# LorenzoFramba/Continual-Learning

Measured on AMD Instinct MI355X. Metric: images/sec UNET 256x256 bs16 train step, higher is better.
Workload: dtype f32; 1 GPU; UNet(21,3,64) 256x256 bs16/GPU fp32 train step (fwd + CE + bwd + Adam), BASELINE.json configs[1]; global_batch=16, parallelism=dp1

## Files before the change

### continual-learning_amd/_lib.py

```python
import ctypes
import os
from ctypes import c_char_p, c_double, c_int, c_longlong, c_size_t, c_void_p

_HERE = os.path.dirname(os.path.abspath(__file__))
LIB_PATH = os.environ.get('CLAMD_LIB') or os.path.join(_HERE, 'libclamd.so')

F32, BF16, SPLIT = 0, 1, 2
WGRAD_CONV3, WGRAD_PW, WGRAD_UP2 = 0, 1, 2

_P, _I, _D, _LL, _SZ = c_void_p, c_int, c_double, c_longlong, c_size_t
OP_CONV3X3, OP_CONV3X3_WINOGRAD, OP_CONV1X1, OP_CONVT2X2_DGRAD, OP_BN_BWD_REDUCE, OP_CONV3X3_WINOGRAD24, OP_CONV3X3_WINOGRAD44 = range(7)


class Tuning(ctypes.Structure):
    _fields_ = [(n, c_int) for n in ('igemm_pws', 'igemm_ws', 'igemm_variant', 'pws_wres', 'wgrad_ws', 'wgrad_dma',
                                     'wgrad_xcd', 'wgrad_blocks', 'wgrad_tw16', 'wino_band', 'wino_persist', 'wino_mt',
                                     'bn_reduce_blocks', 'chsum_blocks', 'cu_reserve', 'wino_half', 'wgrad_streamk')] + [('reserved', c_int * 7)]

    def __init__(self, **kw):
        super().__init__()
        load().clamd_tuning_init(ctypes.byref(self))
        for k, v in kw.items():
            if k not in dict(self._fields_):
                raise KeyError(f'unknown tuning field {k!r}')
            setattr(self, k, int(v))

    def ref(self):
        return ctypes.addressof(self)

    def as_dict(self):
        return {n: getattr(self, n) for n, _ in self._fields_ if n != 'reserved'}


def tune_ptr(t):
    return None if t is None else t.ref()


SIGNATURES = {
    'clamd_last_error': (c_char_p, []),
    'clamd_version': (_I, []),
    'clamd_sizeof_pack_job': (_I, []),
    'clamd_sizeof_adam_tensor': (_I, []),
    'clamd_adam_chunk_elems': (_I, []),
    'clamd_sizeof_importance_tensor': (_I, []),
    'clamd_pack_tile': (_I, []),
    'clamd_bn_bwd_nsums': (_I, []),
    'clamd_sizeof_tuning': (_I, []),
    'clamd_tuning_init': (None, [_P]),
    'clamd_stat_rows': (_I, [_I, _I, _I, _I, _I, _I, _I, _I, _P]),
    'clamd_conv3x3': (_I, [_P, _I, _P, _P, _P, _I, _P, _P, _P, _I, _I, _I, _I, _I, _I, _I, _I, _I, _P, _P]),
    'clamd_conv3x3_border_bias_ok': (_I, [_I, _I, _I, _I, _I, _I, _P]),
    'clamd_conv3x3_bn_sums': (_I, [_I, _I, _I, _I, _I, _I, _P]),
    'clamd_bn_fold_bias': (_I, [_P, _P, _P, _P, _I, _I, _I, _P]),
    'clamd_maxpool2x2': (_I, [_P, _I, _P, _P, _I, _I, _I, _I, _I, _I, _P]),
    'clamd_maxpool2x2_bwd': (_I, [_P, _I, _P, _P, _I, _P, _I, _I, _I, _I, _I, _I, _P]),
    'clamd_bn_fold_pack': (_I, [_I, _P, _I, _I, _I, _P, _I, _P, _P, _P, _I, _I, _I, _P]),
    'clamd_bn_fold_wgrad_pointwise': (_I, [_P, _P, _P, _P, _I, _I, _P]),
    'clamd_bn_fold_wgrad_workspace_bytes': (_SZ, [_I, _I]),
    'clamd_bn_fold_wgrad': (_I, [_P, _I, _P, _P, _P, _P, _P, _SZ, _I, _I, _I, _I, _I, _I, _I, _P]),
    'clamd_conv1x1': (_I, [_P, _I, _P, _P, _P, _I, _P, _P, _P, _I, _I, _I, _I, _I, _I, _I, _I, _P]),
    'clamd_conv1x1_logits': (_I, [_P, _I, _P, _P, _P, _I, _I, _I, _I, _I, _I, _I, _P]),
    'clamd_conv1x1_argmax': (_I, [_P, _I, _P, _P, _P, _P, _I, _I, _I, _I, _I, _I, _I, _P]),
    'clamd_convT2x2_fwd': (_I, [_P, _I, _P, _P, _P, _I, _I, _I, _I, _I, _I, _I, _P]),
    'clamd_convT2x2_dgrad': (_I, [_P, _I, _P, _P, _I, _P, _P, _I, _I, _I, _I, _I, _I, _I, _P]),
    'clamd_wgrad_workspace_bytes': (_SZ, [_I, _I, _I, _I, _I, _I, _I]),
    'clamd_wgrad': (_I, [_I, _P, _I, _P, _I, _P, _SZ, _P, _I, _I, _I, _I, _I, _I, _I, _I, _I, _I, _I, _I, _P, _P]),
    'clamd_bn_finalize': (_I, [_P, _I, _P, _P, _P, _P, _P, _P, _P, _P, _I, _I, _D, _D, _D, _P, _P]),
    'clamd_bn_apply': (_I, [_P, _I, _P, _P, _P, _I, _P, _I, _I, _I, _I, _I, _I, _P]),
    'clamd_bn_bwd_reduce': (_I, [_P, _I, _P, _I, _P, _I, _P, _P, _P, _I, _I, _I, _I, _I, _I, _P, _P]),
    'clamd_bn_bwd_finalize': (_I, [_P, _I, _P, _P, _P, _P, _P, _P, _P, _I, _I, _D, _P]),
    'clamd_bn_bwd_apply': (_I, [_P, _I, _P, _I, _P, _I, _P, _P, _P, _P, _I, _I, _I, _I, _I, _I, _P]),
    'clamd_bn_bwd_apply_sums_rows': (_I, [_I, _I, _I, _I]),
    'clamd_bn_bwd_apply_sums': (_I, [_P, _I, _P, _I, _P, _P, _I, _P, _I, _I, _I, _I, _I, _I, _P]),
    'clamd_rows_sum': (_I, [_P, _I, _P, _I, _I, _P]),
    'clamd_bn_bwd_eval_rows': (_I, [_I, _I, _I, _I, _I]),
    'clamd_bn_bwd_eval': (_I, [_P, _I, _P, _I, _P, _I, _P, _P, _P, _I, _P, _I, _I, _I, _I, _I, _I, _I, _P]),
    'clamd_bn_bwd_eval_finalize': (_I, [_P, _I, _I, _P, _P, _P, _P, _P, _P, _P, _I, _I, _P]),
    'clamd_bn_rows_total': (_I, [_P, _I, _I, _I, _D, _P, _P, _P]),
    'clamd_bn_finalize_total': (_I, [_P, _P, _P, _P, _P, _P, _P, _P, _P, _I, _I, _D, _D, _P, _P]),
    'clamd_bn_bwd_finalize_total': (_I, [_P, _P, _P, _P, _P, _P, _P, _P, _P, _I, _I, _P]),
    'clamd_channel_sum_workspace_bytes': (_SZ, [_I]),
    'clamd_channel_sum': (_I, [_P, _I, _P, _LL, _I, _I, _I, _P, _SZ, _P, _P]),
    'clamd_nchw_to_nhwc': (_I, [_P, _P, _I, _I, _I, _I, _I, _I, _D, _I, _P]),
    'clamd_nhwc_to_nchw': (_I, [_P, _I, _P, _I, _I, _I, _I, _I, _P]),
    'clamd_nchw_im2col3': (_I, [_P, _P, _I, _I, _I, _I, _I, _I, _I, _P]),
    'clamd_pack': (_I, [_P, _I, _I, _I, _P]),
    'clamd_sizeof_wino_pack_job': (_I, []),
    'clamd_wino_pack': (_I, [_P, _I, _I, _P]),
    'clamd_wgrad_winograd_workspace_bytes': (_SZ, [_I, _I]),
    'clamd_wgrad_winograd24_workspace_bytes': (_SZ, [_I, _I]),
    'clamd_wgrad_winograd24': (_I, [_P, _I, _P, _I, _P, _SZ, _P, _I, _I, _I, _I, _I, _I, _I, _I, _I, _I, _I, _P, _P]),
    'clamd_wgrad_winograd': (_I, [_P, _I, _P, _I, _P, _SZ, _P, _I, _I, _I, _I, _I, _I, _I, _I, _I, _I, _I, _P, _P]),
    'clamd_conv3x3_winograd': (_I, [_P, _I, _P, _P, _P, _I, _P, _I, _I, _I, _I, _I, _I, _I, _P, _P]),
    'clamd_wino24_pack': (_I, [_P, _I, _I, _P]),
    'clamd_conv3x3_winograd24': (_I, [_P, _I, _P, _P, _P, _I, _P, _I, _I, _I, _I, _I, _I, _I, _P, _P]),
    'clamd_winograd24_input_elems': (_SZ, [_I, _I, _I, _I]),
    'clamd_winograd24_transform_input': (_I, [_P, _I, _P, _P, _P, _I, _I, _I, _I, _P]),
    'clamd_conv3x3_winograd24_pre': (_I, [_P, _P, _P, _P, _I, _P, _I, _I, _I, _I, _I, _I, _I, _P, _P]),
    'clamd_conv3x3_winograd24_direct_filters': (_I, [_P, _I, _P, _P, _P, _I, _P, _I, _I, _I, _I, _I, _I, _I, _P, _P]),
    'clamd_wgrad_winograd24_pre_operand_elems': (_SZ, [_I, _I, _I, _I]),
    'clamd_wgrad_winograd24_pre_transform': (_I, [_P, _I, _P, _I, _I, _I, _I, _P]),
    'clamd_wgrad_winograd24_pre_workspace_bytes': (_SZ, [_I, _I, _I, _I, _I]),
    'clamd_wgrad_winograd24_pre': (_I, [_P, _I, _P, _P, _P, _SZ, _P, _I, _I, _I, _I, _I, _I, _I, _I, _I, _I, _I, _P, _P]),
    'clamd_wino44_pack': (_I, [_P, _I, _I, _P]),
    'clamd_winograd44_input_elems': (_SZ, [_I, _I, _I, _I]),
    'clamd_winograd44_transform_input': (_I, [_P, _I, _P, _P, _P, _I, _I, _I, _I, _P]),
    'clamd_conv3x3_winograd44_pre': (_I, [_P, _P, _P, _P, _I, _P, _I, _I, _I, _I, _I, _I, _I, _P, _P]),
    'clamd_wgrad_winograd44_pre_operand_elems': (_SZ, [_I, _I, _I, _I]),
    'clamd_wgrad_winograd44_pre_transform': (_I, [_P, _I, _P, _I, _I, _I, _I, _P]),
    'clamd_wgrad_winograd44_pre_workspace_bytes': (_SZ, [_I, _I, _I, _I, _I]),
    'clamd_wgrad_winograd44_pre': (_I, [_P, _I, _P, _P, _P, _SZ, _P, _I, _I, _I, _I, _I, _I, _I, _I, _I, _I, _I, _P, _P]),
    'clamd_ce_workspace_bytes': (_SZ, []),
    'clamd_ce_bad_label_count_offset': (_SZ, []),
    'clamd_ce_fwd_bwd': (_I, [_P, _P, _P, _I, _I, _D, _D, _P, _P, _P, _SZ, _I, _I, _I, _I, _LL, _D, _P]),
    'clamd_ce_count': (_I, [_P, _I, _I, _I, _I, _LL, _P, _SZ, _P]),
    'clamd_ce_fwd_bwd_counted': (_I, [_P, _P, _P, _P, _I, _I, _P, _P, _SZ, _I, _I, _I, _I, _LL, _D, _P]),
    'clamd_ce_unbiased_fwd_bwd': (_I, [_P, _P, _P, _I, _I, _D, _P, _P, _I, _I, _P, _P, _SZ, _I, _I, _I, _I, _LL, _D, _P]),
    'clamd_ce_dice_workspace_bytes': (_SZ, [_I, _I, _I, _I, _I]),
    'clamd_ce_dice_fwd_bwd': (_I, [_P, _P, _P, _P, _I, _I, _P, _P, _SZ, _I, _I, _I, _I, _LL, _D, _D, _D, _I, _I, _I, _D, _P]),
    'clamd_pseudo_entropy_hist': (_I, [_P, _I, _I, _P, _P, _I, _I, _I, _I, _P]),
    'clamd_pseudo_label': (_I, [_P, _I, _I, _P, _P, _P, _P, _P, _D, _I, _I, _I, _LL, _P]),
    'clamd_ce_fwd_bwd_weighted': (_I, [_P, _P, _P, _P, _P, _I, _I, _P, _P, _SZ, _I, _I, _I, _I, _LL, _D, _P]),
    'clamd_pod_workspace_bytes': (_SZ, [_I, _I, _I, _I, _I]),
    'clamd_local_pod_fwd_bwd': (_I, [_P, _I, _P, _I, _I, _I, _I, _I, _I, _D, _P, _P, _P, _SZ, _I, _I, _I, _D, _P]),
    'clamd_class_pixel_counts': (_I, [_P, _P, _P, _I, _I, _I, _I, _LL, _P]),
    'clamd_replay_store': (_I, [_P, _P, _P, _P, _I, _P, _P, _I, _I, _P, _I, _I, _I, _I, _I, _LL, _P]),
    'clamd_replay_mix': (_I, [_P, _P, _I, _P, _P, _I, _I, _P, _P, _I, _P, _P, _P, _I, _I, _I, _LL, _P]),
    'clamd_augment_batch': (_I, [_P, _P, _P, _I, _I, _I, _I, _P, _P, _D, _LL, _P, _P]),
    'clamd_adam_step': (_I, [_P, _P, _I, _P, _P, _P, _P, _P]),
    'clamd_adam_step_consolidated': (_I, [_P, _P, _P, _I, _P, _P, _P, _P, _P, _P]),
    'clamd_importance_accum': (_I, [_P, _P, _I, _D, _D, _I, _P]),
    'clamd_sizeof_sgd_tensor': (_I, []),
    'clamd_sgd_step': (_I, [_P, _P, _P, _I, _P, _P, _P, _P]),
    'clamd_adam_step_tracked': (_I, [_P, _P, _P, _P, _I, _P, _P, _P, _P, _P, _P]),
    'clamd_sgd_step_tracked': (_I, [_P, _P, _P, _P, _I, _P, _P, _P, _P]),
    'clamd_sizeof_path_tensor': (_I, []),
    'clamd_path_importance': (_I, [_P, _P, _I, _D, _D, _P]),
    'clamd_argmax_confusion': (_I, [_P, _P, _P, _P, _I, _I, _I, _I, _I, _P]),
    'clamd_voc_prepare': (_I, [_P, _P, _P, _P, _I, _I, _I, _I, _I, _I, _P, _P]),
    'clamd_label_to_rgb': (_I, [_P, _P, _LL, _LL, _P]),
    'clamd_fill_f32': (_I, [_P, _LL, _D, _P]),
    'clamd_hold_cus': (_I, [_I, _I, _P]),
    'clamd_f32_to_bf16': (_I, [_P, _P, _LL, _P]),
    'clamd_bf16_to_f32': (_I, [_P, _P, _LL, _P]),
    'clamd_scale_by_device_scalar': (_I, [_P, _LL, _P, _P]),
    'clamd_scale_by_device_scalar_nhwc': (_I, [_P, _LL, _I, _P, _P, _LL, _P]),
}

DEBUG_SIGNATURES = {'clamd_debug_hold_cus': (_I, [_I, _I, _P]), 'clamd_debug_mfma_rate': (_LL, [_I, _I, _P, _P])}

_lib = None


def load():
# ... 61 lines not shown
```

### continual-learning_amd/csrc/elementwise.hip

```cpp
#include <initializer_list>
#include <type_traits>
#include "common.hip.h"
#include "clamd_internal.h"

namespace clamd {


constexpr int FIN_THREADS = 256, FIN_CH = 2;
template <int NK>
__device__ inline void sum_partial_rows(const float* __restrict__ rows, int nrows, int Cp, int c0, double* red, double* out) {
    constexpr int COLS = NK * FIN_CH, RL = FIN_THREADS / COLS;
    const int t = threadIdx.x, col = t % COLS, rl = t / COLS;
    if (rl < RL) {
        const float* p = rows + (size_t)(col / FIN_CH) * Cp + c0 + (col % FIN_CH);
        const size_t rs = (size_t)NK * Cp;
        double a0 = 0., a1 = 0., a2 = 0., a3 = 0.;
        int r = rl;
        for (; r + 3 * RL < nrows; r += 4 * RL) {
            a0 += (double)p[(size_t)r * rs]; a1 += (double)p[(size_t)(r + RL) * rs];
            a2 += (double)p[(size_t)(r + 2 * RL) * rs]; a3 += (double)p[(size_t)(r + 3 * RL) * rs];
        }
        for (; r < nrows; r += RL) a0 += (double)p[(size_t)r * rs];
        red[rl * COLS + col] = (a0 + a1) + (a2 + a3);
    }
    __syncthreads();
    if (t < COLS) {
        double v = 0.;
        for (int q = 0; q < RL; ++q) v += red[q * COLS + t];
        out[t] = v;
    }
    __syncthreads();
}

__device__ inline void bn_finalize_channel(bool stats, double s0, double s1, double count, int c, int C, const float* __restrict__ gamma,
                                           const float* __restrict__ beta, float* running_mean, float* running_var, float* scale,
                                           float* shift, float* save_mean, float* save_istd, double momentum, double eps) {
    double mean, var;
    if (stats) {
        mean = s0 / count;
        var = s1 / count - mean * mean;
        var = var > 0. ? var : 0.;
    } else {
        mean = c < C ? (double)running_mean[c] : 0.;
        var = c < C ? (double)running_var[c] : 1.;
    }
    const double istd = 1.0 / sqrt(var + eps);
    const double g = c < C ? (double)gamma[c] : 0., b = c < C ? (double)beta[c] : 0.;
    const float sc = (float)(g * istd);
    scale[c] = sc;
    shift[c] = (float)(b - mean * (g * istd));
    save_mean[c] = (float)mean;
    save_istd[c] = (float)istd;
    if (c < C && running_mean && stats) {
        const double unb = count > 1. ? var * (count / (count - 1.)) : var;
        running_mean[c] = (float)((1. - momentum) * (double)running_mean[c] + momentum * mean);
        running_var[c] = (float)((1. - momentum) * (double)running_var[c] + momentum * unb);
    }
}

__global__ void __launch_bounds__(FIN_THREADS) bn_finalize_kernel(const float* __restrict__ stats, int nrows, const float* __restrict__ gamma,
                                   const float* __restrict__ beta, float* running_mean, float* running_var,
                                   float* scale, float* shift, float* save_mean, float* save_istd,
                                   int Cp, int C, double count, double momentum, double eps, long long* num_batches_tracked) {
    PASS_PRIO();
    __shared__ double red[FIN_THREADS], tot[2 * FIN_CH];
    const int c0 = blockIdx.x * FIN_CH;
    if (stats) sum_partial_rows<2>(stats, nrows, Cp, c0, red, tot);
    if (threadIdx.x >= FIN_CH) return;
    if (num_batches_tracked && stats && blockIdx.x == 0 && threadIdx.x == 0) *num_batches_tracked += 1;
    const int c = c0 + threadIdx.x;
    bn_finalize_channel(stats != nullptr, stats ? tot[threadIdx.x] : 0., stats ? tot[FIN_CH + threadIdx.x] : 0., count, c, C, gamma, beta,
                        running_mean, running_var, scale, shift, save_mean, save_istd, momentum, eps);
}

template <int NK>
__global__ void __launch_bounds__(FIN_THREADS) bn_rows_total_kernel(const float* __restrict__ rows, int nrows, int Cp, double count,
                                                                    double* totals, double* reduce) {
    PASS_PRIO();
    __shared__ double red[FIN_THREADS], tot[NK * FIN_CH];
    const int c0 = blockIdx.x * FIN_CH;
    sum_partial_rows<NK>(rows, nrows, Cp, c0, red, tot);
    if (threadIdx.x >= NK * FIN_CH) return;
    const int k = threadIdx.x / FIN_CH, c = c0 + threadIdx.x % FIN_CH;
    const double v = tot[threadIdx.x];
    if (totals) totals[(size_t)k * Cp + c] = v;
    if (reduce && k < 2) reduce[(size_t)k * Cp + c] = v;
// ... 50 lines not shown
    Vec8<T>::load(ga + pix1 * ga_ldc + cg * 8, g[1]);
    Vec8<T>::load(y + pix1 * y_ldc + cg * 8, v[1]);
    return two;
}

template <typename T, bool POOL>
__global__ void bn_apply_kernel(const T* __restrict__ y, int y_ldc, const float* __restrict__ scale,
                                const float* __restrict__ shift, T* out, int out_ldc, T* pooled, int p_ldc,
                                int B, int H, int W, int Cp) {
    PASS_PRIO();
    const int G = Cp >> 3;
    const long long nitem = POOL ? (long long)B * (H / 2) * (W / 2) * G : (long long)B * H * W * G;
    const long long it0 = (long long)blockIdx.x * blockDim.x + threadIdx.x;
    const int cg = (int)(it0 % G);
    float sc[8], sh[8];
#pragma unroll
    for (int j = 0; j < 8; ++j) { sc[j] = scale[cg * 8 + j]; sh[j] = shift[cg * 8 + j]; }
    for (long long it = it0; it < nitem; it += (long long)gridDim.x * blockDim.x) {
        const long long pix = it / G;
        if constexpr (!POOL) {
            float v[8];
            Vec8<T>::load(y + pix * y_ldc + cg * 8, v);
#pragma unroll
            for (int j = 0; j < 8; ++j) v[j] = __fmaf_rn(v[j], sc[j], sh[j]);
            Vec8<T>::store(out + pix * out_ldc + cg * 8, v);
        } else {
            const PoolWindow win(pix, H, W);
            float m[8];
#pragma unroll
            for (int q = 0; q < 4; ++q) {
                const long long p = win.at(q);
                float v[8];
                Vec8<T>::load(y + p * y_ldc + cg * 8, v);
#pragma unroll
                for (int j = 0; j < 8; ++j) {
                    v[j] = __fmaf_rn(v[j], sc[j], sh[j]);
                    m[j] = (q == 0 || v[j] > m[j]) ? v[j] : m[j];
                }
                Vec8<T>::store(out + p * out_ldc + cg * 8, v);
            }
            Vec8<T>::store(pooled + pix * p_ldc + cg * 8, m);
        }
    }
}

template <typename T, bool BWD>
__global__ void __launch_bounds__(256) maxpool2x2_kernel(const T* __restrict__ x, int x_ldc, T* __restrict__ out, int o_ldc,
                                                        const T* __restrict__ gp, int gp_ldc, const float* __restrict__ sign,
                                                        int B, int H, int W, int Cp) {
    PASS_PRIO();
    const int G = Cp >> 3;
    const long long nitem = (long long)B * (H / 2) * (W / 2) * G;
    for (long long it = (long long)blockIdx.x * blockDim.x + threadIdx.x; it < nitem; it += (long long)gridDim.x * blockDim.x) {
        const int cg = (int)(it % G);
        const long long pix = it / G;
        const PoolWindow win(pix, H, W);
        float m[8], v[4][8];
        int arg[8];
        bool neg[8];
#pragma unroll
        for (int j = 0; j < 8; ++j) neg[j] = sign != nullptr && sign[cg * 8 + j] < 0.f;
#pragma unroll
        for (int q = 0; q < 4; ++q) {
            Vec8<T>::load(x + win.at(q) * x_ldc + cg * 8, v[q]);
#pragma unroll
            for (int j = 0; j < 8; ++j)
                if (q == 0 || (neg[j] ? v[q][j] < m[j] : v[q][j] > m[j])) { m[j] = v[q][j]; arg[j] = q; }
        }
        if constexpr (!BWD) Vec8<T>::store(out + pix * o_ldc + cg * 8, m);
        else {
            float g[8];
            Vec8<T>::load(gp + pix * gp_ldc + cg * 8, g);
#pragma unroll
            for (int q = 0; q < 4; ++q) {
                float o[8];
#pragma unroll
                for (int j = 0; j < 8; ++j) o[j] = arg[j] == q ? g[j] : 0.f;
                Vec8<T>::store(out + win.at(q) * o_ldc + cg * 8, o);
            }
        }
    }
}

template <typename T>
__device__ inline void load_gu(const T* ga, int ga_ldc, const T* gp, int gp_ldc, const T* y, int y_ldc,
                               const float (&sc)[8], const float (&sh)[8], const PoolWindow& win,
                               int cg, float (&g)[4][8], float (&yy)[4][8]) {
    float best[8];
    int arg[8];
#pragma unroll
    for (int q = 0; q < 4; ++q) {
        const long long p = win.at(q);
        Vec8<T>::load(y + p * y_ldc + cg * 8, yy[q]);
        if (ga) Vec8<T>::load(ga + p * ga_ldc + cg * 8, g[q]);
        else {
#pragma unroll
            for (int j = 0; j < 8; ++j) g[q][j] = 0.f;
        }
#pragma unroll
        for (int j = 0; j < 8; ++j) {
            float u = __fmaf_rn(yy[q][j], sc[j], sh[j]);
            if (q == 0 || u > best[j]) { best[j] = u; arg[j] = q; }
        }
    }
    float gpv[8];
    Vec8<T>::load(gp + win.cell() * gp_ldc + cg * 8, gpv);
#pragma unroll
    for (int q = 0; q < 4; ++q)
#pragma unroll
        for (int j = 0; j < 8; ++j) g[q][j] += (arg[j] == q) ? gpv[j] : 0.f;
}

constexpr int NSUM = 5;

__device__ inline void add_five_sums(float (&acc)[NSUM][8], const float (&g)[8], const float (&v)[8]) {
#pragma unroll
    for (int j = 0; j < 8; ++j) {
        const float pos = v[j] > 0.f ? 1.f : 0.f;
        acc[0][j] += g[j]; acc[1][j] += g[j] * v[j]; acc[2][j] += g[j] * pos;
        acc[3][j] += pos; acc[4][j] += v[j];
    }
}

template <typename T, bool POOL>
__global__ void __launch_bounds__(256) bn_bwd_reduce_kernel(const T* __restrict__ ga, int ga_ldc,
                                                            const T* __restrict__ gp, int gp_ldc,
                                                            const T* __restrict__ y, int y_ldc,
                                                            const float* __restrict__ scale,
                                                            const float* __restrict__ shift, float* sums,
                                                            int B, int H, int W, int Cp) {
    PASS_PRIO();
    __shared__ float red[256 * 8];
    const int G = Cp >> 3;
    const int tid = threadIdx.x;
    float acc[NSUM][8];
#pragma unroll
    for (int s = 0; s < NSUM; ++s)
#pragma unroll
        for (int j = 0; j < 8; ++j) acc[s][j] = 0.f;
    const int cg = tid % G;
    const int rows = 256 / G, prow = tid / G;
    {
        float sc[8], sh[8];
        if constexpr (POOL) {
#pragma unroll
            for (int j = 0; j < 8; ++j) { sc[j] = scale[cg * 8 + j]; sh[j] = shift[cg * 8 + j]; }
        }
        const long long npix = POOL ? (long long)B * (H / 2) * (W / 2) : (long long)B * H * W;
        const long long stride = (long long)gridDim.x * rows;
        for (long long pix = (long long)blockIdx.x * rows + prow; pix < npix; pix += POOL ? stride : 2 * stride) {
            if constexpr (!POOL) {
                float g[2][8], v[2][8];
                const bool two = pix + stride < npix;
                const long long pix1 = two ? pix + stride : pix;
                Vec8<T>::load(ga + pix * ga_ldc + cg * 8, g[0]);
                Vec8<T>::load(y + pix * y_ldc + cg * 8, v[0]);
                Vec8<T>::load(ga + pix1 * ga_ldc + cg * 8, g[1]);
                Vec8<T>::load(y + pix1 * y_ldc + cg * 8, v[1]);
#pragma unroll
                for (int u = 0; u < 2; ++u) {
                    if (u == 1 && !two) break;
#pragma unroll
                    for (int j = 0; j < 8; ++j) {
                        const float pos = v[u][j] > 0.f ? 1.f : 0.f;
                        acc[0][j] += g[u][j]; acc[1][j] += g[u][j] * v[u][j]; acc[2][j] += g[u][j] * pos;
                        acc[3][j] += pos; acc[4][j] += v[u][j];
                    }
                }
            } else {
                float g[4][8], v[4][8];
                load_gu<T>(ga, ga_ldc, gp, gp_ldc, y, y_ldc, sc, sh, PoolWindow(pix, H, W), cg, g, v);
#pragma unroll
                for (int q = 0; q < 4; ++q) add_five_sums(acc, g[q], v[q]);
            }
        }
    }
    float* dst = sums + (size_t)blockIdx.x * NSUM * Cp;
    if constexpr (POOL) reduce_block_rows<NSUM>(acc, red, dst, G, Cp, rows);
    else {
#pragma unroll
        for (int s = 0; s < NSUM; ++s) {
            __syncthreads();
#pragma unroll
            for (int j = 0; j < 8; ++j) red[tid * 8 + j] = acc[s][j];
            __syncthreads();
            for (int c = tid; c < Cp; c += 256) {
                const int g8 = c >> 3, j = c & 7;
                float t = 0.f;
                for (int r = 0; r < rows; ++r) t += red[(r * G + g8) * 8 + j];
                dst[s * Cp + c] = t;
            }
        }
    }
// ... 19 lines not shown

__global__ void __launch_bounds__(FIN_THREADS) bn_bwd_finalize_kernel(const float* __restrict__ sums, int nrows, const float* __restrict__ gamma,
                                       const float* __restrict__ save_mean, const float* __restrict__ save_istd,
                                       float* k012, float* dgamma, float* dbeta, float* dbias, int Cp, int C,
                                       double count) {
    PASS_PRIO();
    __shared__ double red[FIN_THREADS], tot[NSUM * FIN_CH];
    const int c0 = blockIdx.x * FIN_CH;
    sum_partial_rows<NSUM>(sums, nrows, Cp, c0, red, tot);
    if (threadIdx.x >= FIN_CH) return;
    const int c = c0 + threadIdx.x;
    double s[NSUM];
#pragma unroll
    for (int k = 0; k < NSUM; ++k) s[k] = tot[k * FIN_CH + threadIdx.x];
    bn_bwd_finalize_channel(s[0], s[1], count, s[0], s[1], s[2], s[3], s[4], c, C, Cp, gamma, save_mean, save_istd, k012, dgamma, dbeta, dbias);
}

__global__ void __launch_bounds__(256) bn_bwd_finalize_total_kernel(const double* __restrict__ totals, const double* __restrict__ reduce,
                                                                    const float* __restrict__ gamma, const float* __restrict__ save_mean,
                                                                    const float* __restrict__ save_istd, float* k012, float* dgamma,
                                                                    float* dbeta, float* dbias, int Cp, int C) {
    PASS_PRIO();
    const int c = blockIdx.x * blockDim.x + threadIdx.x;
    if (c >= Cp) return;
    const double* t = totals + c;
    const double s2 = dbias ? t[2 * (size_t)Cp] : 0., s3 = dbias ? t[3 * (size_t)Cp] : 0., s4 = dbias ? t[4 * (size_t)Cp] : 0.;
    bn_bwd_finalize_channel(reduce[c], reduce[Cp + c], reduce[2 * Cp], t[0], t[Cp], s2, s3, s4, c, C, Cp, gamma, save_mean, save_istd,
                            k012, dgamma, dbeta, dbias);
}

__device__ inline float bn_bwd_gz(float k0, float k1, float k2, float g, float y) { return fmaf(k0, g, fmaf(k1, y, k2)); }


__device__ inline void load_k012(const float* k012, int Cp, int cg, float (&k0)[8], float (&k1)[8], float (&k2)[8]) {
#pragma unroll
    for (int j = 0; j < 8; ++j) {
        k0[j] = k012[cg * 8 + j]; k1[j] = k012[Cp + cg * 8 + j]; k2[j] = k012[2 * Cp + cg * 8 + j];
    }
}

template <typename T, bool POOL>
__global__ void bn_bwd_apply_kernel(const T* __restrict__ ga, int ga_ldc, const T* __restrict__ gp, int gp_ldc,
                                    const T* __restrict__ y, int y_ldc, const float* __restrict__ scale,
                                    const float* __restrict__ shift, const float* __restrict__ k012, T* gz,
                                    int gz_ldc, int B, int H, int W, int Cp) {
    PASS_PRIO();
    const int G = Cp >> 3;
    const long long nitem = POOL ? (long long)B * (H / 2) * (W / 2) * G : (long long)B * H * W * G;
    const long long it0 = (long long)blockIdx.x * blockDim.x + threadIdx.x;
    float k0[8], k1[8], k2[8];
    if constexpr (!POOL) {
        const int cg = (int)(it0 % G);
        load_k012(k012, Cp, cg, k0, k1, k2);
        for (long long it = it0; it < nitem; it += (long long)gridDim.x * blockDim.x) {
            const long long pix = it / G;
            float g[8], v[8];
            Vec8<T>::load(ga + pix * ga_ldc + cg * 8, g);
            Vec8<T>::load(y + pix * y_ldc + cg * 8, v);
#pragma unroll
            for (int j = 0; j < 8; ++j) g[j] = v[j] > 0.f ? bn_bwd_gz(k0[j], k1[j], k2[j], g[j], v[j]) : 0.f;
            Vec8<T>::store(gz + pix * gz_ldc + cg * 8, g);
        }
    } else {
        for (long long it = it0; it < nitem; it += (long long)gridDim.x * blockDim.x) {
            const int cg = (int)(it % G);
            const long long pix = it / G;
            load_k012(k012, Cp, cg, k0, k1, k2);
            float sc[8], sh[8];
#pragma unroll
            for (int j = 0; j < 8; ++j) { sc[j] = scale[cg * 8 + j]; sh[j] = shift[cg * 8 + j]; }
            const PoolWindow win(pix, H, W);
            float g[4][8], v[4][8];
            load_gu<T>(ga, ga_ldc, gp, gp_ldc, y, y_ldc, sc, sh, win, cg, g, v);
#pragma unroll
            for (int q = 0; q < 4; ++q) {
#pragma unroll
                for (int j = 0; j < 8; ++j) g[q][j] = v[q][j] > 0.f ? bn_bwd_gz(k0[j], k1[j], k2[j], g[q][j], v[q][j]) : 0.f;
                Vec8<T>::store(gz + win.at(q) * gz_ldc + cg * 8, g[q]);
            }
        }
    }
}

template <typename T>
__global__ void __launch_bounds__(256) bn_bwd_apply_sums_kernel(const T* __restrict__ ga, int ga_ldc, const T* __restrict__ y, int y_ldc,
                                                                const float* __restrict__ k012, T* gz, int gz_ldc, float* rows,
                                                                long long npix, int Cp) {
    PASS_PRIO();
    __shared__ float red[256 * 8];
    const int G = Cp >> 3;
    const long long nitem = npix * G;
    const long long it0 = (long long)blockIdx.x * 256 + threadIdx.x;
    const int cg = (int)(it0 % G);
    float k0[8], k1[8], k2[8], acc[1][8] = {};
    load_k012(k012, Cp, cg, k0, k1, k2);
    for (long long it = it0; it < nitem; it += (long long)gridDim.x * 256) {
        const long long pix = it / G;
        float g[8], v[8];
        Vec8<T>::load(ga + pix * ga_ldc + cg * 8, g);
        Vec8<T>::load(y + pix * y_ldc + cg * 8, v);
#pragma unroll
        for (int j = 0; j < 8; ++j) {
            g[j] = v[j] > 0.f ? bn_bwd_gz(k0[j], k1[j], k2[j], g[j], v[j]) : 0.f;
            acc[0][j] += g[j];
        }
        Vec8<T>::store(gz + pix * gz_ldc + cg * 8, g);
    }
    reduce_block_rows<1>(acc, red, rows + (size_t)blockIdx.x * Cp, G, Cp, 256 / G);
}

constexpr int NSUM_EVAL = 3;

__device__ inline void add_eval_sums(float (&acc)[NSUM_EVAL][8], const float (&sc)[8], int nlive, float (&g)[8], const float (&v)[8]) {
#pragma unroll
    for (int j = 0; j < 8; ++j) {
        const float o = (v[j] > 0.f && j < nlive) ? sc[j] * g[j] : 0.f;
        acc[0][j] += g[j]; acc[1][j] += g[j] * v[j]; acc[2][j] += o;
        g[j] = o;
    }
}

template <typename T, bool POOL>
__global__ void __launch_bounds__(256) bn_bwd_eval_kernel(const T* __restrict__ ga, int ga_ldc, const T* __restrict__ gp, int gp_ldc,
                                                          const T* __restrict__ y, int y_ldc, const float* __restrict__ scale,
                                                          const float* __restrict__ shift, T* __restrict__ gz, int gz_ldc, float* rows,
                                                          int B, int H, int W, int Cp, int C) {
    PASS_PRIO();
    __shared__ float red[256 * 8];
    const int G = Cp >> 3, tid = threadIdx.x;
    const int cg = tid % G, prow = tid / G, per = 256 / G;
    const int nlive = C - cg * 8;
    float sc[8], acc[NSUM_EVAL][8];
#pragma unroll
    for (int j = 0; j < 8; ++j) {
        sc[j] = scale[cg * 8 + j];
#pragma unroll
        for (int s = 0; s < NSUM_EVAL; ++s) acc[s][j] = 0.f;
    }
    const long long npix = POOL ? (long long)B * (H / 2) * (W / 2) : (long long)B * H * W;
    const long long stride = (long long)gridDim.x * per;
    if constexpr (!POOL) {
        for (long long pix = (long long)blockIdx.x * per + prow; pix < npix; pix += 2 * stride) {
            float g[2][8], v[2][8];
            long long pix1;
            const bool two = load_pixel_pair<T>(ga, ga_ldc, y, y_ldc, pix, stride, npix, cg, pix1, g, v);
            add_eval_sums(acc, sc, nlive, g[0], v[0]);
            Vec8<T>::store(gz + pix * gz_ldc + cg * 8, g[0]);
            if (two) {
                add_eval_sums(acc, sc, nlive, g[1], v[1]);
                Vec8<T>::store(gz + pix1 * gz_ldc + cg * 8, g[1]);
            }
        }
    } else {
        float sh[8];
#pragma unroll
        for (int j = 0; j < 8; ++j) sh[j] = shift[cg * 8 + j];
        for (long long pix = (long long)blockIdx.x * per + prow; pix < npix; pix += stride) {
            const PoolWindow win(pix, H, W);
            float g[4][8], v[4][8];
            load_gu<T>(ga, ga_ldc, gp, gp_ldc, y, y_ldc, sc, sh, win, cg, g, v);
#pragma unroll
            for (int q = 0; q < 4; ++q) {
#pragma unroll
                for (int j = 0; j < 8; ++j) {
                    const float o = (v[q][j] > 0.f && j < nlive) ? sc[j] * g[q][j] : 0.f;
                    acc[0][j] += g[q][j]; acc[1][j] += g[q][j] * v[q][j]; acc[2][j] += o;
// ... 206 lines not shown
        }
        Vec8<T>::store(dst + pix * ldc + cg * 8, o);
    }
}

template <typename T>
__global__ void nhwc_to_nchw_kernel(const T* __restrict__ src, int ldc, float* dst, int B, int C, int H, int W) {
    const long long hw = (long long)H * W, n = (long long)B * C * hw;
    for (long long it = (long long)blockIdx.x * blockDim.x + threadIdx.x; it < n;
         it += (long long)gridDim.x * blockDim.x) {
        const long long p = it % hw;
        const int c = (int)((it / hw) % C);
        const long long b = it / (hw * C);
        dst[it] = ld1<T>(src + (b * hw + p) * ldc + c);
    }
}

static inline long long reduce_grid_cap(int forced, int Cp, int lo, int hi, int budget) {
    if (forced > 0) return forced;
    long long c = budget / Cp;
    return c < lo ? lo : (c > hi ? hi : c);
}

}

using namespace clamd;

static inline long long grid_rows(long long items, long long per, long long cap) {
    const long long g = (items + per - 1) / per;
    return g > cap ? cap : (g < 1 ? 1 : g);
}
static inline int ew_grid(long long nitem, int cap = 4096) { return (int)grid_rows(nitem, 256, cap); }
static bool pow2_channels(int Cp) { return Cp >= 32 && Cp <= 2048 && (Cp & (Cp - 1)) == 0; }
static const char POW2_RULE[] = "physical channels must be a power of two in [32,2048]";
static inline long long pass_pixels(int B, int H, int W, bool pooled) { return pooled ? (long long)B * (H / 2) * (W / 2) : (long long)B * H * W; }
static inline int pixel_rows(int Cp) { return 256 / (Cp / 8) > 0 ? 256 / (Cp / 8) : 1; }

long long clamd_bn_bwd_reduce_rows(int B, int H, int W, int Cp, bool pooled, const clamd_tuning& tn) {
    return grid_rows(pass_pixels(B, H, W, pooled), pixel_rows(Cp), reduce_grid_cap(tn.bn_reduce_blocks, Cp, 256, 1024, 131072));
}
constexpr int CHSUM_MAX_BLOCKS = 1024;

template <typename T> struct Tag { using type = T; };
template <typename F>
static bool dispatch(int dtype, bool flag, F&& f) {
    auto with_flag = [&](auto tag) { if (flag) f(tag, std::true_type{}); else f(tag, std::false_type{}); };
    if (dtype == CLAMD_BF16) with_flag(Tag<bf16_t>{});
    else if (dtype == CLAMD_F32) with_flag(Tag<float>{});
    else if (dtype == CLAMD_SPLIT) with_flag(Tag<split_t>{});
    else return false;
    return true;
}
template <typename F>
static bool dispatch(int dtype, F&& f) { return dispatch(dtype, false, [&](auto tag, auto) { f(tag); }); }

static int fail(const char* name, const char* text) {
    static thread_local char msg[256];
    snprintf(msg, sizeof(msg), "%s: %s", name, text);
    return clamd_fail(msg);
}

enum Need { OPTIONAL, REQUIRED, SOURCE };
constexpr int NO_PITCH = 0x7fffffff;
struct TensorArg { const void* p; int ldc; Need need; };
static int check_streaming(const char* name, bool channels_ok, const char* channel_rule, int Cp, long long B, long long H, long long W,
                           bool pooled, int dtype, std::initializer_list<TensorArg> tensors) {
    if (!channels_ok) return fail(name, channel_rule);
    if (B <= 0 || H <= 0 || W <= 0) return fail(name, "bad sizes");
    if (pooled && ((H | W) & 1)) return fail(name, "pooling needs even H, W");
    bool has_source = false, any_source = false;
    for (const TensorArg& t : tensors) {
        if (t.need == REQUIRED && !t.p) return fail(name, "null argument");
        if (t.need == SOURCE) { any_source = true; has_source |= t.p != nullptr; }
    }
    if (any_source && !has_source) return fail(name, "no gradient source (ga and gp are both a null argument)");
    for (const TensorArg& t : tensors)
        if (t.p && t.ldc < Cp) return fail(name, "pitches must be >= Cp");
    for (const TensorArg& t : tensors)
        if (t.ldc != NO_PITCH)
            if (int e = clamd_check_split(dtype, t.p, t.ldc)) return e;
    return 0;
}

extern "C" {

int clamd_bn_finalize(const float* stats, int stat_rows, const float* gamma, const float* beta, float* running_mean,
                      float* running_var, float* scale, float* shift, float* save_mean, float* save_istd,
                      int Cp, int C, double count, double momentum, double eps, long long* num_batches_tracked, void* stream) {
    if (Cp <= 0 || Cp % 8 || C > Cp) return clamd_fail("bn_finalize: bad channel counts");
    if (stats && stat_rows <= 0) return clamd_fail("bn_finalize: stat_rows must be the row count the producing launch wrote");
    if (!scale || !shift || !save_mean || !save_istd || (C > 0 && (!gamma || !beta))) return clamd_fail("bn_finalize: null argument");
    if (!stats && C > 0 && (!running_mean || !running_var)) return clamd_fail("bn_finalize: eval mode (stats == NULL) needs the running statistics");
    if (!running_mean != !running_var) return clamd_fail("bn_finalize: running_mean and running_var go together");
    hipLaunchKernelGGL(bn_finalize_kernel, dim3(Cp / FIN_CH), dim3(FIN_THREADS), 0, (hipStream_t)stream, stats, stat_rows, gamma,
                       beta, running_mean, running_var, scale, shift, save_mean, save_istd, Cp, C, count, momentum, eps, num_batches_tracked);
    return clamd_check_launch("bn_finalize");
}

int clamd_bn_rows_total(const float* rows, int nrows, int nk, int Cp, double count, double* totals, double* reduce, void* stream) {
    if (Cp <= 0 || Cp % 8) return clamd_fail("bn_rows_total: bad channel count");
    if (!rows || nrows <= 0) return clamd_fail("bn_rows_total: nrows must be the row count the producing launch wrote");
    if (!totals && !reduce) return clamd_fail("bn_rows_total: nothing to write");
    if (!(count > 0.)) return clamd_fail("bn_rows_total: count must be positive");
    hipStream_t s = (hipStream_t)stream;
    if (nk == 2)
        hipLaunchKernelGGL(bn_rows_total_kernel<2>, dim3(Cp / FIN_CH), dim3(FIN_THREADS), 0, s, rows, nrows, Cp, count, totals, reduce);
    else if (nk == NSUM)
        hipLaunchKernelGGL(bn_rows_total_kernel<NSUM>, dim3(Cp / FIN_CH), dim3(FIN_THREADS), 0, s, rows, nrows, Cp, count, totals, reduce);
    else return clamd_fail("bn_rows_total: nk must be 2 (statistics rows) or 5 (clamd_bn_bwd_nsums rows)");
    return clamd_check_launch("bn_rows_total");
}

int clamd_bn_finalize_total(const double* reduce, const float* gamma, const float* beta, float* running_mean, float* running_var,
                            float* scale, float* shift, float* save_mean, float* save_istd, int Cp, int C, double momentum, double eps,
                            long long* num_batches_tracked, void* stream) {
    if (Cp <= 0 || Cp % 8 || C <= 0 || C > Cp) return clamd_fail("bn_finalize_total: bad channel counts");
    if (!reduce || !gamma || !beta || !scale || !shift || !save_mean || !save_istd) return clamd_fail("bn_finalize_total: null argument");
    if (!running_mean != !running_var) return clamd_fail("bn_finalize_total: running_mean and running_var go together");
    hipLaunchKernelGGL(bn_finalize_total_kernel, dim3((Cp + 255) / 256), dim3(256), 0, (hipStream_t)stream, reduce, gamma, beta, running_mean,
                       running_var, scale, shift, save_mean, save_istd, Cp, C, momentum, eps, num_batches_tracked);
    return clamd_check_launch("bn_finalize_total");
}

int clamd_bn_apply(const void* y, int y_ldc, const float* scale, const float* shift, void* out, int out_ldc,
                   void* pooled, int p_ldc, int B, int H, int W, int Cp, int dtype, void* stream) {
    if (int e = check_streaming("bn_apply", pow2_channels(Cp), POW2_RULE, Cp, B, H, W, pooled != nullptr, dtype,
                                {{y, y_ldc, REQUIRED}, {scale, NO_PITCH, REQUIRED}, {shift, NO_PITCH, REQUIRED}, {out, out_ldc, REQUIRED},
                                 {pooled, p_ldc, OPTIONAL}}))
        return e;
    const dim3 g(ew_grid(pass_pixels(B, H, W, pooled != nullptr) * (Cp / 8), 8192)), b(256);
    const bool ok = dispatch(dtype, pooled != nullptr, [&](auto tag, auto pool) {
        using T = typename decltype(tag)::type;
        hipLaunchKernelGGL((bn_apply_kernel<T, decltype(pool)::value>), g, b, 0, (hipStream_t)stream, (const T*)y, y_ldc, scale, shift,
                           (T*)out, out_ldc, (T*)pooled, p_ldc, B, H, W, Cp);
    });
    return ok ? clamd_check_launch("bn_apply") : fail("bn_apply", "bad dtype");
}

static int launch_maxpool(const char* name, bool bwd, const void* x, int x_ldc, void* out, int o_ldc, const void* gp, int gp_ldc,
                          const float* sign, int B, int H, int W, int Cp, int dtype, void* stream) {
    if (int e = check_streaming(name, Cp > 0 && Cp % 8 == 0, "physical channels must be a positive multiple of 8", Cp, B, H, W, true, dtype,
                                {{x, x_ldc, REQUIRED}, {out, o_ldc, REQUIRED}, {gp, gp_ldc, bwd ? REQUIRED : OPTIONAL}}))
        return e;
    const dim3 g(ew_grid(pass_pixels(B, H, W, true) * (Cp / 8), 8192)), b(256);
    const bool ok = dispatch(dtype, bwd, [&](auto tag, auto back) {
        using T = typename decltype(tag)::type;
        hipLaunchKernelGGL((maxpool2x2_kernel<T, decltype(back)::value>), g, b, 0, (hipStream_t)stream, (const T*)x, x_ldc, (T*)out, o_ldc,
                           (const T*)gp, gp_ldc, sign, B, H, W, Cp);
    });
    return ok ? clamd_check_launch(name) : fail(name, "bad dtype");
}

int clamd_maxpool2x2(const void* x, int x_ldc, const float* sign, void* pooled, int p_ldc, int B, int H, int W, int Cp, int dtype, void* stream) {
    return launch_maxpool("maxpool2x2", false, x, x_ldc, pooled, p_ldc, nullptr, 0, sign, B, H, W, Cp, dtype, stream);
}

int clamd_maxpool2x2_bwd(const void* x, int x_ldc, const float* sign, const void* gp, int gp_ldc, void* gx, int gx_ldc, int B, int H, int W, int Cp,
                         int dtype, void* stream) {
    return launch_maxpool("maxpool2x2_bwd", true, x, x_ldc, gx, gx_ldc, gp, gp_ldc, sign, B, H, W, Cp, dtype, stream);
}

int clamd_bn_bwd_reduce(const void* ga, int ga_ldc, const void* gp, int gp_ldc, const void* y, int y_ldc,
                        const float* scale, const float* shift, float* sums, int sum_rows, int B, int H, int W, int Cp,
                        int dtype, const clamd_tuning* tune, void* stream) {
    const Need pool_only = gp ? REQUIRED : OPTIONAL;
    if (int e = check_streaming("bn_bwd_reduce", pow2_channels(Cp), POW2_RULE, Cp, B, H, W, gp != nullptr, dtype,
                                {{ga, ga_ldc, SOURCE}, {gp, gp_ldc, SOURCE}, {y, y_ldc, REQUIRED}, {sums, NO_PITCH, REQUIRED},
                                 {scale, NO_PITCH, pool_only}, {shift, NO_PITCH, pool_only}}))
        return e;
    if (int e = clamd_check_tuning(tune)) return e;
    const long long nrows = clamd_bn_bwd_reduce_rows(B, H, W, Cp, gp != nullptr, clamd_tune(tune));
    if (sum_rows != nrows) return fail("bn_bwd_reduce", "sum_rows does not match clamd_stat_rows(CLAMD_OP_BN_BWD_REDUCE, ...)");
    const bool ok = dispatch(dtype, gp != nullptr, [&](auto tag, auto pool) {
        using T = typename decltype(tag)::type;
        hipLaunchKernelGGL((bn_bwd_reduce_kernel<T, decltype(pool)::value>), dim3((unsigned)nrows), dim3(256), 0, (hipStream_t)stream,
                           (const T*)ga, ga_ldc, (const T*)gp, gp_ldc, (const T*)y, y_ldc, scale, shift, sums, B, H, W, Cp);
    });
    return ok ? clamd_check_launch("bn_bwd_reduce") : fail("bn_bwd_reduce", "bad dtype");
}

int clamd_bn_bwd_finalize(const float* sums, int sum_rows, const float* gamma, const float* save_mean, const float* save_istd,
                          float* k012, float* dgamma, float* dbeta, float* dbias, int Cp, int C, double count,
                          void* stream) {
    if (Cp <= 0 || Cp % 8 || C > Cp) return clamd_fail("bn_bwd_finalize: bad channel counts");
    if (sum_rows <= 0) return clamd_fail("bn_bwd_finalize: sum_rows must be the row count the producing launch wrote");
    if (!sums || !save_mean || !save_istd || !k012 || (C > 0 && (!gamma || !dgamma || !dbeta))) return clamd_fail("bn_bwd_finalize: null argument");
    hipLaunchKernelGGL(bn_bwd_finalize_kernel, dim3(Cp / FIN_CH), dim3(FIN_THREADS), 0, (hipStream_t)stream, sums, sum_rows,
                       gamma, save_mean, save_istd, k012, dgamma, dbeta, dbias, Cp, C, count);
    return clamd_check_launch("bn_bwd_finalize");
}

int clamd_bn_bwd_finalize_total(const double* totals, const double* reduce, const float* gamma, const float* save_mean,
                                const float* save_istd, float* k012, float* dgamma, float* dbeta, float* dbias, int Cp, int C, void* stream) {
    if (Cp <= 0 || Cp % 8 || C <= 0 || C > Cp) return clamd_fail("bn_bwd_finalize_total: bad channel counts");
    if (!totals || !reduce || !gamma || !save_mean || !save_istd || !k012 || !dgamma || !dbeta)
        return clamd_fail("bn_bwd_finalize_total: null argument");
    hipLaunchKernelGGL(bn_bwd_finalize_total_kernel, dim3((Cp + 255) / 256), dim3(256), 0, (hipStream_t)stream, totals, reduce, gamma,
                       save_mean, save_istd, k012, dgamma, dbeta, dbias, Cp, C);
    return clamd_check_launch("bn_bwd_finalize_total");
}

int clamd_bn_bwd_apply(const void* ga, int ga_ldc, const void* gp, int gp_ldc, const void* y, int y_ldc,
                       const float* scale, const float* shift, const float* k012, void* gz, int gz_ldc, int B,
                       int H, int W, int Cp, int dtype, void* stream) {
    const Need pool_only = gp ? REQUIRED : OPTIONAL;
    if (int e = check_streaming("bn_bwd_apply", pow2_channels(Cp), POW2_RULE, Cp, B, H, W, gp != nullptr, dtype,
                                {{ga, ga_ldc, SOURCE}, {gp, gp_ldc, SOURCE}, {y, y_ldc, REQUIRED}, {k012, NO_PITCH, REQUIRED},
                                 {gz, gz_ldc, REQUIRED}, {scale, NO_PITCH, pool_only}, {shift, NO_PITCH, pool_only}}))
        return e;
    const dim3 g(ew_grid(pass_pixels(B, H, W, gp != nullptr) * (Cp / 8), 8192)), b(256);
    const bool ok = dispatch(dtype, gp != nullptr, [&](auto tag, auto pool) {
        using T = typename decltype(tag)::type;
        hipLaunchKernelGGL((bn_bwd_apply_kernel<T, decltype(pool)::value>), g, b, 0, (hipStream_t)stream, (const T*)ga, ga_ldc,
                           (const T*)gp, gp_ldc, (const T*)y, y_ldc, scale, shift, k012, (T*)gz, gz_ldc, B, H, W, Cp);
    });
    return ok ? clamd_check_launch("bn_bwd_apply") : fail("bn_bwd_apply", "bad dtype");
}

static long long apply_sums_rows(long long npix, int Cp) { return grid_rows(npix * (Cp / 8), 256, 2048); }

int clamd_bn_bwd_apply_sums_rows(int B, int H, int W, int Cp) {
    if (B <= 0 || H <= 0 || W <= 0 || !pow2_channels(Cp)) return clamd_fail("bn_bwd_apply_sums_rows: bad sizes");
    return (int)apply_sums_rows((long long)B * H * W, Cp);
}

int clamd_bn_bwd_apply_sums(const void* ga, int ga_ldc, const void* y, int y_ldc, const float* k012, void* gz, int gz_ldc,
                            float* gz_rows, int nrows, int B, int H, int W, int Cp, int dtype, void* stream) {
    if (int e = check_streaming("bn_bwd_apply_sums", pow2_channels(Cp), POW2_RULE, Cp, B, H, W, false, dtype,
                                {{ga, ga_ldc, REQUIRED}, {y, y_ldc, REQUIRED}, {k012, NO_PITCH, REQUIRED}, {gz, gz_ldc, REQUIRED},
                                 {gz_rows, NO_PITCH, REQUIRED}}))
        return e;
    const long long npix = (long long)B * H * W;
    if (nrows != apply_sums_rows(npix, Cp)) return fail("bn_bwd_apply_sums", "nrows must be clamd_bn_bwd_apply_sums_rows(B, H, W, Cp)");
    const bool ok = dispatch(dtype, [&](auto tag) {
        using T = typename decltype(tag)::type;
        hipLaunchKernelGGL((bn_bwd_apply_sums_kernel<T>), dim3((unsigned)nrows), dim3(256), 0, (hipStream_t)stream, (const T*)ga, ga_ldc,
                           (const T*)y, y_ldc, k012, (T*)gz, gz_ldc, gz_rows, npix, Cp);
    });
    return ok ? clamd_check_launch("bn_bwd_apply_sums") : fail("bn_bwd_apply_sums", "bad dtype");
}

static long long eval_rows(int B, int H, int W, int Cp, bool pooled) {
    return grid_rows(pass_pixels(B, H, W, pooled), pixel_rows(Cp), reduce_grid_cap(0, Cp, 256, 2048, 262144));
}

int clamd_bn_bwd_eval_rows(int B, int H, int W, int Cp, int pooled) {
    if (B <= 0 || H <= 0 || W <= 0 || !pow2_channels(Cp)) return clamd_fail("bn_bwd_eval_rows: bad sizes");
    if (pooled && ((H | W) & 1)) return clamd_fail("bn_bwd_eval_rows: pooling needs even H, W");
    return (int)eval_rows(B, H, W, Cp, pooled != 0);
}

int clamd_bn_bwd_eval(const void* ga, int ga_ldc, const void* gp, int gp_ldc, const void* y, int y_ldc, const float* scale, const float* shift,
                      void* gz, int gz_ldc, float* rows, int nrows, int B, int H, int W, int Cp, int C, int dtype, void* stream) {
    if (int e = check_streaming("bn_bwd_eval", pow2_channels(Cp) && C > 0 && C <= Cp,
                                "physical channels must be a power of two in [32,2048], 0 < C <= Cp", Cp, B, H, W, gp != nullptr, dtype,
                                {{ga, ga_ldc, SOURCE}, {gp, gp_ldc, SOURCE}, {y, y_ldc, REQUIRED}, {scale, NO_PITCH, REQUIRED},
                                 {gz, gz_ldc, REQUIRED}, {rows, NO_PITCH, REQUIRED}, {shift, NO_PITCH, gp ? REQUIRED : OPTIONAL}}))
        return e;
    if (nrows != eval_rows(B, H, W, Cp, gp != nullptr)) return fail("bn_bwd_eval", "nrows must be clamd_bn_bwd_eval_rows(B, H, W, Cp, gp != NULL)");
    const bool ok = dispatch(dtype, gp != nullptr, [&](auto tag, auto pool) {
        using T = typename decltype(tag)::type;
        hipLaunchKernelGGL((bn_bwd_eval_kernel<T, decltype(pool)::value>), dim3((unsigned)nrows), dim3(256), 0, (hipStream_t)stream,
                           (const T*)ga, ga_ldc, (const T*)gp, gp_ldc, (const T*)y, y_ldc, scale, shift, (T*)gz, gz_ldc, rows, B, H, W, Cp, C);
    });
    return ok ? clamd_check_launch("bn_bwd_eval") : fail("bn_bwd_eval", "bad dtype");
}

int clamd_bn_bwd_eval_finalize(const float* rows, int nrows, int nsums, const float* scale, const float* save_mean, const float* save_istd,
                               float* k012, float* dgamma, float* dbeta, float* dbias, int Cp, int C, void* stream) {
    if (Cp <= 0 || Cp % 8 || C <= 0 || C > Cp) return clamd_fail("bn_bwd_eval_finalize: bad channel counts");
    if (!rows || nrows <= 0) return clamd_fail("bn_bwd_eval_finalize: nrows must be the row count the producing launch wrote");
    if (!scale || !save_mean || !save_istd || !dgamma || !dbeta) return clamd_fail("bn_bwd_eval_finalize: null argument");
    hipStream_t s = (hipStream_t)stream;
    if (nsums == NSUM_EVAL)
        hipLaunchKernelGGL(bn_bwd_eval_finalize_kernel<NSUM_EVAL>, dim3(Cp / FIN_CH), dim3(FIN_THREADS), 0, s, rows, nrows, scale, save_mean,
                           save_istd, k012, dgamma, dbeta, dbias, Cp, C);
    else if (nsums == NSUM)
        hipLaunchKernelGGL(bn_bwd_eval_finalize_kernel<NSUM>, dim3(Cp / FIN_CH), dim3(FIN_THREADS), 0, s, rows, nrows, scale, save_mean,
                           save_istd, k012, dgamma, dbeta, dbias, Cp, C);
    else return clamd_fail("bn_bwd_eval_finalize: nsums must be 3 (clamd_bn_bwd_eval rows) or 5 (clamd_bn_bwd_nsums rows)");
    return clamd_check_launch("bn_bwd_eval_finalize");
}

int clamd_rows_sum(const float* rows, int nrows, float* out, int Cp, int C, void* stream) {
    if (!rows || !out || nrows <= 0 || Cp <= 0 || Cp % 8 || C > Cp) return clamd_fail("rows_sum: bad arguments");
    hipLaunchKernelGGL(channel_sum_final_kernel, dim3(Cp / FIN_CH), dim3(FIN_THREADS), 0, (hipStream_t)stream, rows, nrows, out, Cp, C);
    return clamd_check_launch("rows_sum");
}

size_t clamd_channel_sum_workspace_bytes(int Cp) { return (size_t)CHSUM_MAX_BLOCKS * (Cp > 0 ? Cp : 0) * sizeof(float); }

int clamd_channel_sum(const void* g, int ldc, float* out, long long npix, int Cp, int C, int dtype, float* workspace,
                      size_t ws_bytes, const clamd_tuning* tune, void* stream) {
    if (pow2_channels(Cp) && C > Cp) return clamd_fail("channel_sum: bad sizes");
    if (int e = check_streaming("channel_sum", pow2_channels(Cp), POW2_RULE, Cp, 1, 1, npix, false, dtype,
                                {{g, ldc, REQUIRED}, {out, NO_PITCH, REQUIRED}}))
        return e;
    if (int e = clamd_check_tuning(tune)) return e;
    const long long gb = grid_rows(npix, pixel_rows(Cp), reduce_grid_cap(clamd_tune(tune).chsum_blocks, Cp, 256, CHSUM_MAX_BLOCKS, 131072));
    if (!workspace || (size_t)gb * Cp * sizeof(float) > ws_bytes) return clamd_fail("channel_sum: workspace too small (clamd_channel_sum_workspace_bytes)");
    hipStream_t s = (hipStream_t)stream;
// ... 77 lines not shown
```

### continual-learning_amd/csrc/wino24g.hip

```cpp
#include <string.h>
#include <algorithm>
#include "common.hip.h"
#include "clamd_internal.h"
#include "wino_common.hip.h"

namespace clamd {

struct W24XformParams {
    const float* x; int x_ldc;
    const float* scale; const float* shift;
    float* v;
    int B, H, W, Kp;
};

#define W24G_COLS(t_, o_)                                                                                          \
    do {                                                                                                           \
        _Pragma("unroll") for (int e_ = 0; e_ < 4; ++e_) {                                                         \
            const float t0_ = t_[0][e_], t1_ = t_[1][e_], t2_ = t_[2][e_], t3_ = t_[3][e_], t4_ = t_[4][e_], t5_ = t_[5][e_]; \
            const float pq_ = fmaf(-4.f, t2_, t4_), qq_ = fmaf(-4.f, t1_, t3_);                                    \
            const float rr_ = t4_ - t2_, ss_ = t3_ - t1_;                                                          \
            o_[0][e_] = fmaf(4.f, t0_, fmaf(-5.f, t2_, t4_));                                                      \
            o_[1][e_] = pq_ + qq_; o_[2][e_] = pq_ - qq_;                                                          \
            o_[3][e_] = fmaf(2.f, ss_, rr_); o_[4][e_] = fmaf(-2.f, ss_, rr_);                                     \
            o_[5][e_] = fmaf(4.f, t1_, fmaf(-5.f, t3_, t5_));                                                      \
// ... 531 lines not shown
            const int n = n0 + 32 * nt + 4 * ng;
            float4 bias4 = make_float4(0.f, 0.f, 0.f, 0.f);
            if (p.bias && n < p.Np) bias4 = *reinterpret_cast<const float4*>(p.bias + (CLS ? 4 * p.Np : 0) + n);
            float4 bm1 = bias4;
            if (edge_tile && n < p.Np) {
                const int ya = y0 + 2 * (tl / TXN);
                bias4 = *reinterpret_cast<const float4*>(p.bias + ((ya == 0 ? 0 : (ya == p.H - 1 ? 6 : 3)) + 1) * p.Np + n);
                bm1 = *reinterpret_cast<const float4*>(p.bias + ((ya + 1 == p.H - 1 ? 6 : 3) + 1) * p.Np + n);
            }
#pragma unroll
            for (int q = 0; q < 4; ++q) {
                float4 R[4];
#pragma unroll
                for (int i = 0; i < 4; ++i) R[i] = *reinterpret_cast<const float4*>(exb + ((i * 4 + q) * 32 + tl) * W24G_EXP + 4 * ng);
#pragma unroll
                for (int pp = 0; pp < 2; ++pp) {
                    float4 o;
                    if (pp == 0) {
                        o.x = R[0].x + R[1].x + R[2].x; o.y = R[0].y + R[1].y + R[2].y;
                        o.z = R[0].z + R[1].z + R[2].z; o.w = R[0].w + R[1].w + R[2].w;
                    } else {
                        o.x = R[1].x - R[2].x - R[3].x; o.y = R[1].y - R[2].y - R[3].y;
                        o.z = R[1].z - R[2].z - R[3].z; o.w = R[1].w - R[2].w - R[3].w;
                    }
                    const int yy = y0 + 2 * oty + pp, xx = x0 + 4 * otx + q;
                    if (!plain) {
                        float4 b4 = pp ? bm1 : bias4;
                        if (edge_tile && n < p.Np && (q == 0 || q == 3) && (xx == 0 || xx == p.W - 1))
                            b4 = *reinterpret_cast<const float4*>(p.bias + border_class(yy, xx, p.H, p.W) * p.Np + n);
                        o.x = fmaxf(o.x + b4.x, relu_lo); o.y = fmaxf(o.y + b4.y, relu_lo);
                        o.z = fmaxf(o.z + b4.z, relu_lo); o.w = fmaxf(o.w + b4.w, relu_lo);
                    }
                    if (!RAGGED || (yy < p.H && xx < p.W)) {
                        *reinterpret_cast<float4*>(p.y + (((size_t)b * p.H + yy) * p.W + xx) * p.y_ldc + n) = o;
                        if (!plain) {
                            st1[nt][0] += o.x; st1[nt][1] += o.y; st1[nt][2] += o.z; st1[nt][3] += o.w;
                            st2[nt][0] = fmaf(o.x, o.x, st2[nt][0]); st2[nt][1] = fmaf(o.y, o.y, st2[nt][1]);
                            st2[nt][2] = fmaf(o.z, o.z, st2[nt][2]); st2[nt][3] = fmaf(o.w, o.w, st2[nt][3]);
                        }
                    }
                }
            }
        }
        if (rows_base) { cur_tn = tn; cur_tm = tm; }
        __syncthreads();
    }
    if (cur_tn >= 0) fold_stats();
}

struct W24WgXformParams {
    const float* src; int ldc;
    float* dst;
    int B, H, W, Rp, Tp;
};

template <int TXN>
__global__ void __launch_bounds__(256) wino24g_wgrad_xform_kernel(const W24WgXformParams p) {
    SIDE_PRIO();
    constexpr int TYN = 32 / TXN, PW = 4 * TXN, PH = 2 * TYN;
    const int ng = p.Rp >> 2;
    const long long total = (long long)p.Tp * ng;
    const int tiles_x = (p.W + PW - 1) / PW, tiles_y = (p.H + PH - 1) / PH;
    const unsigned img = (unsigned)p.H * (unsigned)p.W * (unsigned)p.ldc * 4u;
    const size_t ps = (size_t)p.Tp * p.Rp;
    for (long long idx = (long long)blockIdx.x * 256 + threadIdx.x; idx < total; idx += (long long)gridDim.x * 256) {
        const int g = (int)(idx % ng);
        const int t = (int)(idx / ng);
        const int tm = t >> 5, r = t & 31;
        const int x0 = (tm % tiles_x) * PW + 4 * (r % TXN), y0 = ((tm / tiles_x) % tiles_y) * PH + 2 * (r / TXN), b = tm / (tiles_x * tiles_y);
        float* const dst = p.dst + (size_t)t * p.Rp + 4 * g;
        const __amdgpu_buffer_rsrc_t rs = make_rsrc((const char*)p.src + (size_t)b * img, img);
        float gq[2][4][4];
#pragma unroll
        for (int a = 0; a < 2; ++a)
#pragma unroll
            for (int q = 0; q < 4; ++q) {
                const int yy = y0 + a, xx = x0 + q;
                const uint4 u = buf_ld16(rs, (yy < p.H && xx < p.W) ? (unsigned)(((yy * p.W + xx) * p.ldc + 4 * g) * 4) : BUF_OOB, 0u);
                gq[a][q][0] = __uint_as_float(u.x); gq[a][q][1] = __uint_as_float(u.y);
                gq[a][q][2] = __uint_as_float(u.z); gq[a][q][3] = __uint_as_float(u.w);
            }
#pragma unroll
        for (int i = 0; i < 4; ++i) {
            float z[4][4], o[6][4];
#pragma unroll
            for (int q = 0; q < 4; ++q)
#pragma unroll
                for (int e = 0; e < 4; ++e)
                    z[q][e] = i == 0 ? gq[0][q][e] : (i == 1 ? gq[0][q][e] + gq[1][q][e] : (i == 2 ? gq[0][q][e] - gq[1][q][e] : -gq[1][q][e]));
#pragma unroll
            for (int e = 0; e < 4; ++e) {
                const float sa = z[0][e] + z[2][e], sb = z[1][e] + z[3][e], sc = fmaf(4.f, z[2][e], z[0][e]), sd = fmaf(4.f, z[3][e], z[1][e]);
                o[0][e] = z[0][e]; o[1][e] = sa + sb; o[2][e] = sa - sb;
                o[3][e] = fmaf(2.f, sd, sc); o[4][e] = fmaf(-2.f, sd, sc); o[5][e] = z[3][e];
            }
#pragma unroll
            for (int j = 0; j < 6; ++j) *reinterpret_cast<float4*>(dst + (6 * i + j) * ps) = make_float4(o[j][0], o[j][1], o[j][2], o[j][3]);
        }
    }
}

struct W24WgGemmParams {
    const float* yt;
    const float* v;
    float* partial;
    int Rp, Cp, Tp, nsplit, tiles_per_split;
    int npl;
};

constexpr int W24G_D = 8;

__global__ void __launch_bounds__(256, 1) wino24g_wgrad_kernel(const W24WgGemmParams p) {
    int tid = threadIdx.x;
    const int lane = tid & 63;
    const int w = __builtin_amdgcn_readfirstlane(tid >> 6);
    const int i32 = lane & 31, h = lane >> 5;
    const int rb_n = p.Rp >> 8, cb_n = p.Cp >> 8;
    int bid = xcd_remap(blockIdx.x, gridDim.x);
    const int cb = bid % cb_n; bid /= cb_n;
    const int rb = bid % rb_n; bid /= rb_n;
    const int split = bid % p.nsplit;
    const int pl = bid / p.nsplit;
    const int r0 = rb * 256 + (w >> 1) * 128, c0 = cb * 256 + (w & 1) * 128;
    const int t_begin = split * p.tiles_per_split;
    const int t_end = min(p.Tp, t_begin + p.tiles_per_split);
    const int nsteps = max(t_end - t_begin, 0) >> 1;

    const int nk = p.Cp >> 3;
    const unsigned a_bytes = (unsigned)p.Tp * (unsigned)p.Rp * 4u;
    const __amdgpu_buffer_rsrc_t ars = make_rsrc((const char*)p.yt + (size_t)pl * a_bytes, a_bytes);
    const __amdgpu_buffer_rsrc_t brs = make_rsrc(p.v, (unsigned)((size_t)(p.Tp >> 5) * nk * p.npl * 1024));
    const __amdgpu_buffer_rsrc_t ars_dead = make_rsrc(p.yt, 0u), brs_dead = make_rsrc(p.v, 0u);
    const unsigned a_vo = (unsigned)((h * p.Rp + r0 + 4 * i32) * 4);
    const unsigned b_vo = (unsigned)(((c0 >> 3) + (i32 >> 1)) * p.npl * 1024 + (i32 & 1) * 512 + h * 16);
    const unsigned a_step = (unsigned)p.Rp * 8u;
    const unsigned a_so0 = (unsigned)t_begin * (unsigned)p.Rp * 4u;
    const unsigned b_blk = (unsigned)nk * (unsigned)p.npl * 1024u, b_pl = (unsigned)pl * 1024u;

    f32x16 acc[4][4];
#pragma unroll
    for (int m = 0; m < 4; ++m)
#pragma unroll
        for (int n = 0; n < 4; ++n)
#pragma unroll
            for (int e = 0; e < 16; ++e) acc[m][n][e] = 0.f;

    uint4 a[W24G_D], b[W24G_D];
    auto load = [&](int d, int s) {
        const bool live = s < nsteps;
        const unsigned t = (unsigned)(t_begin + 2 * s);
        a[d] = buf_ld16(live ? ars : ars_dead, a_vo, a_so0 + (unsigned)s * a_step);
        b[d] = buf_ld16(live ? brs : brs_dead, b_vo, (t >> 5) * b_blk + b_pl + (t & 31u) * 16u);
    };
#pragma unroll
    for (int d = 0; d < W24G_D; ++d) {
        load(d, d);
        asm volatile("" ::: "memory");
    }
    for (int s0 = 0; s0 < nsteps; s0 += W24G_D) {
#pragma unroll
        for (int d = 0; d < W24G_D; ++d) {
            const float am[4] = {__uint_as_float(a[d].x), __uint_as_float(a[d].y), __uint_as_float(a[d].z), __uint_as_float(a[d].w)};
            const float bn[4] = {__uint_as_float(b[d].x), __uint_as_float(b[d].y), __uint_as_float(b[d].z), __uint_as_float(b[d].w)};
#pragma unroll
            for (int m = 0; m < 4; ++m)
#pragma unroll
                for (int n = 0; n < 4; ++n) acc[m][n] = __builtin_amdgcn_mfma_f32_32x32x2f32(am[m], bn[n], acc[m][n], 0, 0, 0);
            load(d, s0 + d + W24G_D);
            __builtin_amdgcn_sched_group_barrier(0x008, 16, 0);
            __builtin_amdgcn_sched_group_barrier(0x020, 2, 0);
        }
    }

    float* const out = p.partial + (((size_t)split * p.npl + pl) * p.Rp) * (size_t)p.Cp;
#pragma unroll
    for (int m = 0; m < 4; ++m)
#pragma unroll
// ... 640 lines not shown
```

### continual-learning_amd/csrc/wino44g.hip

```cpp
#include <string.h>
#include <algorithm>
#include "common.hip.h"
#include "clamd_internal.h"
#include "wino_common.hip.h"

namespace clamd {

#ifdef CLAMD_DIAG
__device__ unsigned long long g_w44_diag[8];
#define W44_T() __builtin_amdgcn_s_memtime()
#define W44_ADD(i_, v_) do { if (threadIdx.x == 0) atomicAdd(&g_w44_diag[i_], (unsigned long long)(v_)); } while (0)
#else
#define W44_T() 0ull
#define W44_ADD(i_, v_) do { } while (0)
#endif

__device__ inline void w44_bt6(const float (&t)[6], float (&o)[6]) {
    const float pq = fmaf(-4.f, t[2], t[4]), qq = fmaf(-4.f, t[1], t[3]);
    const float rr = t[4] - t[2], ss = t[3] - t[1];
    o[0] = fmaf(4.f, t[0], fmaf(-5.f, t[2], t[4]));
    o[1] = pq + qq; o[2] = pq - qq;
    o[3] = fmaf(2.f, ss, rr); o[4] = fmaf(-2.f, ss, rr);
    o[5] = fmaf(4.f, t[1], fmaf(-5.f, t[3], t[5]));
}
__device__ inline void w44_a6(const float (&z)[4], float (&o)[6]) {
    const float sa = z[0] + z[2], sb = z[1] + z[3], sc = fmaf(4.f, z[2], z[0]), sd = fmaf(4.f, z[3], z[1]);
    o[0] = z[0]; o[1] = sa + sb; o[2] = sa - sb;
    o[3] = fmaf(2.f, sd, sc); o[4] = fmaf(-2.f, sd, sc); o[5] = z[3];
}
__device__ inline void w44_gt6(const float (&t)[6], float (&o)[3]) {
    const float s12 = t[1] + t[2], d12 = t[2] - t[1], s34 = t[3] + t[4], d34 = t[3] - t[4];
    o[0] = 0.25f * t[0] - (1.f / 6.f) * s12 + (1.f / 24.f) * s34;
    o[1] = (1.f / 6.f) * d12 + (1.f / 12.f) * d34;
    o[2] = -(1.f / 6.f) * s12 + (1.f / 6.f) * s34 + t[5];
}


struct W44XformParams {
    const float* x; int x_ldc;
    const float* scale; const float* shift;
    float* v;
    int B, H, W, Kp;
};

template <int TXN>
__global__ void __launch_bounds__(256) wino44_xform_kernel(const W44XformParams p) {
    PASS_PRIO();
    constexpr int TYN = 32 / TXN, PW = 4 * TXN, PH = 4 * TYN;
    constexpr int HPH = PH / 2;
    constexpr int HW_ = PW + 2, HH_ = HPH + 2, PIX = HW_ * HH_;
    constexpr int PITCH = 9;
    constexpr int NJ = (PIX * 8 + 255) / 256;
    __shared__ uint4 sm[PIX * PITCH];
    const int tid = threadIdx.x, lane = tid & 63, w = tid >> 6;
    const int nk = p.Kp >> 3;
    const int tiles_x = (p.W + PW - 1) / PW, tiles_y = (p.H + PH - 1) / PH;
    const int nth = 2 * tiles_x * tiles_y * p.B;
    const int bid = xcd_remap(blockIdx.x, gridDim.x);
    const int kg = bid / nth, tmh = bid - kg * nth;
    const int tm = tmh >> 1, s = tmh & 1;
    const int x0 = (tm % tiles_x) * PW, y0 = ((tm / tiles_x) % tiles_y) * PH + s * HPH, b = tm / (tiles_x * tiles_y);
    const unsigned img = (unsigned)p.H * (unsigned)p.W * (unsigned)p.x_ldc * 4u;
    const __amdgpu_buffer_rsrc_t xrs = make_rsrc((const char*)p.x + (size_t)b * img, img);
    {
        const int g = tid & 7;
        const int ch = kg * 32 + 4 * g;
        const bool chan_ok = ch < p.Kp;
        float4 sc = make_float4(1.f, 1.f, 1.f, 1.f), sh = make_float4(0.f, 0.f, 0.f, 0.f);
        if (p.scale && chan_ok) { sc = *reinterpret_cast<const float4*>(p.scale + ch); sh = *reinterpret_cast<const float4*>(p.shift + ch); }
#pragma unroll
        for (int j = 0; j < NJ; ++j) {
            const int pix = (tid >> 3) + 32 * j;
            if (pix < PIX) {
                const int hy = pix / HW_, hx = pix - hy * HW_;
                const int yy = y0 + hy - 1, xx = x0 + hx - 1;
                const bool ok = chan_ok && yy >= 0 && yy < p.H && xx >= 0 && xx < p.W;
                const uint4 u = buf_ld16(xrs, ok ? (unsigned)(((yy * p.W + xx) * p.x_ldc + ch) * 4) : BUF_OOB, 0u);
                float4 f = make_float4(__uint_as_float(u.x), __uint_as_float(u.y), __uint_as_float(u.z), __uint_as_float(u.w));
                if (p.scale) {
                    f.x = ok ? fmaf(f.x, sc.x, sh.x) : 0.f; f.y = ok ? fmaf(f.y, sc.y, sh.y) : 0.f;
                    f.z = ok ? fmaf(f.z, sc.z, sh.z) : 0.f; f.w = ok ? fmaf(f.w, sc.w, sh.w) : 0.f;
                }
                sm[pix * PITCH + g] = make_uint4(__float_as_uint(f.x), __float_as_uint(f.y), __float_as_uint(f.z), __float_as_uint(f.w));
            }
        }
    }
    __syncthreads();
    const int kc = kg * 4 + w;
    if (kc >= nk) return;
    const int r16 = lane & 15, h = (lane >> 4) & 1, rh = lane >> 5;
    const int ty = r16 / TXN, tx = r16 % TXN;
    const uint4* const src = sm + ((4 * ty) * HW_ + 4 * tx) * PITCH + 2 * w + h;
    float t[3][6][4];
#pragma unroll
    for (int c = 0; c < 6; ++c) {
        float d[6][4];
#pragma unroll
        for (int a = 0; a < 6; ++a) {
            const uint4 u = src[(a * HW_ + c) * PITCH];
            d[a][0] = __uint_as_float(u.x); d[a][1] = __uint_as_float(u.y); d[a][2] = __uint_as_float(u.z); d[a][3] = __uint_as_float(u.w);
        }
#pragma unroll
        for (int e = 0; e < 4; ++e) {
            const float col[6] = {d[0][e], d[1][e], d[2][e], d[3][e], d[4][e], d[5][e]};
            float o[6];
            w44_bt6(col, o);
            t[0][c][e] = rh ? o[3] : o[0]; t[1][c][e] = rh ? o[4] : o[1]; t[2][c][e] = rh ? o[5] : o[2];
        }
    }
    const int r = 16 * s + r16;
    float* const dst = p.v + (((size_t)tm * nk + kc) * 36 + 18 * rh) * 256 + h * 128 + r * 4;
// ... 526 lines not shown
```

### continual-learning_amd/csrc/wino_common.hip.h

```cpp
#pragma once
#include <stdio.h>
#include <algorithm>
#include <type_traits>
#include "common.hip.h"
#include "clamd_internal.h"

namespace clamd {

struct WinoParams {
    const float* x; int x_ldc;
    const float* w;
    const float* bias;
    float* y; int y_ldc;
    float* stats;
    int B, H, W, Kp, Np, relu;
    int band;
    int nblk;
    int bias_classes = 0;
};

struct WinoPackJob {
    const float* w; float* dst;
    int Np, Kp, N, K;
    int n_seg0, n_seg0p, k_seg0, k_seg0p;
    int dgrad;
    int block0;
    const float* kscale;
};

__device__ inline int wn_phys2log(int p, int seg0, int seg0p, int L) {
    if (p < seg0p) return p < seg0 ? p : -1;
    const int l = seg0 + (p - seg0p);
    return l < L ? l : -1;
}

struct WinoReduceParams {
    const float* partial; float* out;
    int nsplit, Rp, Cp, R, C, r_seg0, r_seg0p, c_seg0, c_seg0p;
};

inline int wino_fail(const char* who, const char* what) {
    char msg[256];
    snprintf(msg, sizeof(msg), "%s: %s", who, what);
    return clamd_fail(msg);
}

struct WinoTile { int ph, pw; };
inline WinoTile wino_tile(int W, int rows) { return W >= 32 ? WinoTile{rows, 32} : WinoTile{2 * rows, 16}; }
inline WinoTile w24_tile(int W) { return wino_tile(W, 8); }
inline WinoTile w44_block(int W) { return wino_tile(W, 16); }
inline long long wino_tiles(WinoTile t, int B, int H, int W) { return (long long)B * ((H + t.ph - 1) / t.ph) * ((W + t.pw - 1) / t.pw); }

inline long long wino_stat_rows(long long tiles, int Cout_p, int slab, int wg_per_cu, const clamd_tuning& tn) {
    const long long nblk = tiles * ((Cout_p + slab - 1) / slab), cap = (long long)wg_per_cu * clamd_usable_cus(tn);
    return (tn.wino_persist && nblk > cap) ? cap : tiles;
}

int wino_band(long long tiles, long long slabs, double x_elems, double f_elems, int forced);

struct WinoGrid { unsigned grid; bool ragged; };
int wino_forward_plan(WinoParams& p, WinoTile t, long long slabs, double x_elems, double f_elems, long long grid_cap, int stat_rows,
                      long long want_rows, const clamd_tuning& tn, const char* who, const char* op, WinoGrid* g);

template <class F>
inline void wino_dispatch(bool wide, bool ragged, bool cls, F&& launch) {
    auto pick = [](bool b, auto&& f) { if (b) f(std::true_type{}); else f(std::false_type{}); };
    pick(wide, [&](auto w) { pick(ragged, [&](auto r) { pick(cls, [&](auto c) { launch(w, r, c); }); }); });
}

int wino_wgrad_nsplit(int ntiles, int blocks, const clamd_tuning& tn, int* per);
inline int wino_wgrad_max_split(int blocks) { return std::max(1, 512 / blocks); }

using WinoPackKernel = void (*)(const WinoPackJob*, int, int, const FoldBias);
int wino_launch_pack(WinoPackKernel kernel, const char* who, const void* jobs_dev, int njobs, int total_blocks, const FoldBias* fold, hipStream_t stream);

#ifdef CLAMD_DIAG
#define CLAMD_DIAG_READER(fn_, sym_, n_)                                                                                   \
    int fn_(unsigned long long* out, int reset) {                                                                          \
        if (hipMemcpyFromSymbol(out, HIP_SYMBOL(sym_), 8 * (n_)) != hipSuccess) return -1;                                 \
        if (reset) { unsigned long long z[n_] = {0}; if (hipMemcpyToSymbol(HIP_SYMBOL(sym_), z, 8 * (n_)) != hipSuccess) return -1; } \
        return 0;                                                                                                          \
    }
#endif

long long clamd_winograd24_stat_rows(int B, int H, int W, int Cout_p, const clamd_tuning& tn);
int launch_wino24(WinoParams p, const clamd_tuning& tn, int stat_rows, hipStream_t stream);
long long clamd_winograd44_stat_rows(int B, int H, int W, int Cout_p, const clamd_tuning& tn);
long long clamd_winograd24_half_stat_rows(int B, int H, int W, int Cout_p, const clamd_tuning& tn);
int launch_wino24_half(WinoParams p, const clamd_tuning& tn, int stat_rows, hipStream_t stream);

struct WinoPreForm {
    const char* name;
    const char* op;
    const char* hw_rule;
    const char* tile_note;
    int planes;
    int hmask;
    WinoTile (*tile)(int W);
    int xform_wgs;
    double band_x;
    int cin_mult, cin_min, y_mult;
    bool y_bound;
    const char* yt_launch;
    long long (*stat_rows)(int B, int H, int W, int Cout_p, const clamd_tuning& tn);
    void (*launch_xform)(bool wide, unsigned grid, hipStream_t s, const float* x, int x_ldc, const float* scale, const float* shift, float* v,
                         int B, int H, int W, int Cp);
    void (*launch_conv)(bool wide, bool ragged, unsigned grid, hipStream_t s, const WinoParams& p);
    void (*launch_yt)(bool wide, unsigned grid, hipStream_t s, const float* gz, int gz_ldc, float* yt, int B, int H, int W, int Rp, int Tp);
    void (*launch_reduce)(int phs, unsigned grid, hipStream_t s, const WinoReduceParams& p);
};
size_t wino_pre_input_elems(const WinoPreForm& f, int B, int H, int W, int Cp);
int wino_pre_transform_input(const WinoPreForm& f, const float* x, int x_ldc, const float* scale, const float* shift, float* v, int B, int H, int W,
                             int Cp, void* stream);
int wino_pre_conv3x3(const WinoPreForm& f, const float* v, const float* w_wino, const float* bias, float* y, int y_ldc, float* stats, int stat_rows,
                     int B, int H, int W, int Cin_p, int Cout_p, int relu, const clamd_tuning* tune, void* stream);
size_t wino_pre_operand_elems(const WinoPreForm& f, int B, int H, int W, int Rp);
size_t wino_pre_workspace_bytes(const WinoPreForm& f, int B, int H, int W, int Rp, int Cp);
// ... 7 lines not shown
```

### continual-learning_amd/engine.py

```python
import weakref

import torch
import torch.nn as nn

from . import _lib, bnops, syncbn, unet as U
from ._lib import call, ptr, tune_ptr
from .ops import PackTable, WinoPackTable, cpad
from .plan import ALGOS, plan_net

_SIDE_STREAMS = {}


def _side_stream(dev, n):
    key = (dev.index if dev.index is not None else torch.cuda.current_device(), n)
    if key not in _SIDE_STREAMS:
        _SIDE_STREAMS[key] = torch.cuda.Stream(device=dev)
    return _SIDE_STREAMS[key]


def _timed(tag, flops, nbytes, unit, name, *args):
    kt = U.KERNEL_TIMING
    if kt is None:
        call(name, *args)
        return
# ... 98 lines not shown
            self._ev_early.record(self.wg)
        else:
            for t in wino_late:
                t.run(sp)
        self._ev_pack_late, self._pack_late_pending = None, pack_late is not None

    def release_late_pack(self):
        if not self._pack_late_pending:
            return
        self._pack_late_pending = False
        if not self._single() and self.late_on_side:
            ev = torch.cuda.Event()
            ev.record(torch.cuda.current_stream())
            self.wg.wait_event(ev)
            self._late.run(self._dcode, self.wg.cuda_stream)
            self._ev_pack_late = torch.cuda.Event()
            self._ev_pack_late.record(self.wg)
        else:
            self._late.run(self._dcode, _lib.stream_ptr())

    def need_late_pack(self):
        self.release_late_pack()
        if self._ev_pack_late is not None:
            torch.cuda.current_stream().wait_event(self._ev_pack_late)
            self._ev_pack_late = None

    def need_wino_filters(self, u):
        if self._pack_pending == 2 and (u.level >= 1 or u.pack_late):
            torch.cuda.current_stream().wait_event(self._ev_early)
            self.wg.wait_stream(torch.cuda.current_stream())
            for t in self._wino_late:
                t.run(self.wg.cuda_stream)
            self._pack_pending = 1
        if self._pack_pending == 1 and u.pack_late:
            torch.cuda.current_stream().wait_stream(self.wg)
            self._pack_pending = 0

    def join_forward(self):
        if self._pack_pending == 2:
            for t in self._wino_late:
                t.run(self.wg.cuda_stream)
        if self._pack_pending:
            torch.cuda.current_stream().wait_stream(self.wg)
            self._pack_pending = 0
        self.need_late_pack()

    def start_backward(self, rccl):
        self._wg_used = self._x3_fold = False
        self._pack_pending = 0
        self._yt_ev, self._x3_ev = [None, None], None
        self._third = self.x3 is not None and not self._single()
        if self._third and rccl:
            from . import ddp
            self._third = ddp.hw_queues(self.dev) >= 8
        self._third = self._third and not torch.cuda.is_current_stream_capturing()

    def param_grad_stream(self):
        if self._single():
            return _lib.stream_ptr()
        self.wg.wait_stream(torch.cuda.current_stream())
        self._wg_used = True
        return self.wg.cuda_stream

    def gradient_stream(self):
        return self.wg if self._wg_used else None

    def wgrad_transform_stream(self, bufs):
        if not self._third:
            return None, None
        self._yt_flip ^= 1
        self._x3_buf = bufs[self._yt_flip]
        self.x3.wait_stream(torch.cuda.current_stream())
        if self._yt_ev[self._yt_flip] is not None:
            self.x3.wait_event(self._yt_ev[self._yt_flip])
        return self.x3.cuda_stream, self._x3_buf

    def wgrad_transformed(self):
        self._x3_ev = torch.cuda.Event()
        self._x3_ev.record(self.x3)

    def wgrad_after_transform(self):
        self.wg.wait_event(self._x3_ev)

    def wgrad_operand_read(self):
        self._yt_ev[self._yt_flip], self._x3_ev = torch.cuda.Event(), None
        self._yt_ev[self._yt_flip].record(self.wg)

    def fold_fixup_stream(self, sw):
        if not self._third:
            return sw
        ev = torch.cuda.Event()
        ev.record(self.wg)
        self.x3.wait_event(ev)
        self._x3_fold = True
        return self.x3.cuda_stream

    def join_stage(self):
        if self._x3_fold:
            self.wg.wait_stream(self.x3)
            self._x3_fold = False

    def join_backward(self):
        self.join_stage()
        if self._wg_used:
            torch.cuda.current_stream().wait_stream(self.wg)


class _Engine:
    @property
    def model(self):
        return self._model_ref()

    def __init__(self, model, B, H, W, device):
        lib = _lib.load()
        self._model_ref = weakref.ref(model)
        self.B, self.H, self.W, self.dev = B, H, W, device
        self.dcode, self.tdtype = U._DTYPES[model.compute_dtype]
        self.pack_late_at = int(U.PACK_LATE_AT)
        self.tuning = model.tuning
        self.NS = lib.clamd_bn_bwd_nsums()
        self.generation = 0
        self.dl_src = None
        self.fwd_modes = ()
        self.bn_group = None
        self._has_sync = None
        self._sync_arena = None
        self.esize = 2 if self.dcode == _lib.BF16 else 4
        K, d = model.num_classes, model.conv_dim
        self.K, self.Kp = K, cpad(K)
        T = self.tdtype
        dev = device

        def act(level, c):
            return torch.zeros(B, H >> level, W >> level, c, dtype=T, device=dev)

        named = dict(model.named_parameters())
        bufs = dict(model.named_buffers())
        mods = dict(model.named_modules())
        self.param_names = [n for n, _ in model.named_parameters()]
        sizes = [named[n].numel() for n in self.param_names]
        self.gflat = torch.zeros(sum(sizes), dtype=torch.float32, device=dev)
        self.goffset, self.gshape, off = {}, {}, 0
        for n in reversed(self.param_names):
            k = named[n].numel()
            self.goffset[n] = (off, k)
            self.gshape[n] = tuple(named[n].shape)
            off += k

        self.x_in = act(0, cpad(model.in_dim))
        self.stages = []
        C = [d, 2 * d, 4 * d, 8 * d]
        self.cat = [act(l, 2 * cpad(C[l])) for l in range(4)]
        self.gcat = [act(l, 2 * cpad(C[l])) for l in range(4)]
        self.pool = [act(l + 1, cpad(C[l])) for l in range(4)]
        self.gpool = [act(l + 1, cpad(C[l])) for l in range(4)]

        def unit(prefix, ci, bi, p, xin):
            u = _Unit()
            u.plan, u.name = p, p.name
            u.f, u.d, u.g = ALGOS[p.fwd], p.dgrad and ALGOS[p.dgrad], ALGOS[p.wgrad]
            u.w, u.b = named[f'{prefix}.{ci}.weight'], named[f'{prefix}.{ci}.bias']
            u.gamma, u.beta = named[f'{prefix}.{bi}.weight'], named[f'{prefix}.{bi}.bias']
            u.rm, u.rv = bufs[f'{prefix}.{bi}.running_mean'], bufs[f'{prefix}.{bi}.running_var']
            u.nbt = bufs[f'{prefix}.{bi}.num_batches_tracked']
            u.bn, u.bn_train = mods[f'{prefix}.{bi}'], True
            u.bn_parent, u.bn_parent_name, u.bn_key, u.bn_sync = mods[prefix], prefix, str(bi), False
            u.keys = (f'{prefix}.{ci}.weight', f'{prefix}.{ci}.bias', f'{prefix}.{bi}.weight', f'{prefix}.{bi}.bias')
# ... 22 lines not shown
            (c0, b0, _, mid), (c1, b1, _, _) = st['convs']
            pa, pb = next(plans), next(plans)
            k = pa.level
            if i > 4:
                xin, g_in = self.cat[k], self.gcat[k]
            ua = act(k, cpad(mid))
            a, b = unit(pre, c0, b0, pa, xin), unit(pre, c1, b1, pb, ua)
            a.out, a.pooled, a.g_in = ua, None, g_in
            b.g_in = act(k, cpad(mid))
            a.g_src = (b.g_in, b.g_in.shape[-1], None)
            if st['tail'] is None:
                b.out, b.pooled = self.cat[k], self.pool[k]
                b.g_src = (self.gcat[k], self.gcat[k].shape[-1], self.gpool[k])
                a.out_ldc, b.out_ldc = a.out.shape[-1], b.out.shape[-1]
                xin, g_in = self.pool[k], self.gpool[k]
                self.stages.append(dict(kind='enc', convs=(a, b)))
                continue
            b.out, b.pooled, g_ub = act(k, cpad(mid)), None, act(k, cpad(mid))
            b.g_src = (g_ub, g_ub.shape[-1], None)
            a.out_ldc, b.out_ldc = a.out.shape[-1], b.out.shape[-1]
            kind, ti, tcin, tcout = st['tail']
            tail = tails[f'{pre}.{ti}'] = _Tail()
            tail.w, tail.b = named[f'{pre}.{ti}.weight'], named[f'{pre}.{ti}.bias']
            tail.keys = (f'{pre}.{ti}.weight', f'{pre}.{ti}.bias')
            tail.cin, tail.cin_p, tail.cout, tail.cout_p = tcin, cpad(tcin), tcout, cpad(tcout)
            tail.kind, tail.x, tail.g_x, tail.level = kind, b.out, g_ub, k
            taps = 4 if kind == 'convT' else 1
            tail.wf = torch.zeros(taps * tail.cout_p * tail.cin_p, dtype=T, device=dev)
            tail.wd = torch.zeros(tail.cin_p * taps * tail.cout_p, dtype=T, device=dev)
            if kind == 'convT':
                up = self.cat[k - 1]
                tail.y_slice = up[..., tail.cout_p:]
                tail.gy_slice = self.gcat[k - 1][..., tail.cout_p:]
                tail.y_ldc = up.shape[-1]
            else:
                self.dl = act(0, self.Kp)
            tail.bias_p = torch.zeros(tail.cout_p, dtype=torch.float32, device=dev)
            self.stages.append(dict(kind='dec', convs=(a, b), tail=tail))
        self.convs = convs = [u for st in self.stages for u in st['convs']]
        self.tails = list(tails.values())
        by = {u.name: u for u in convs}
        for u in convs:
            p = u.plan
            if p.sums_by is not None:
                u.sum_src = by.get(p.sums_by) or tails[p.sums_by]
                u.sum_src.consumer = u
            if p.fold_src is not None:
                u.fold_src = by[p.fold_src]
                u.fold_src.apply_folded = True
            if p.fold_a is not None:
                u.fold_a = by[p.fold_a]
            if p.pool_fold is not None:
                k, (nxt, dec) = u.level, (by[n] for n in p.pool_fold)
                u.pool_fold, u.apply_in_filters, u.y, u.y_ldc = True, True, self.cat[k], self.cat[k].shape[-1]
                comp = torch.zeros(2, dec.cin_p, dtype=torch.float32, device=dev)
                comp[0, u.cout_p:] = 1.0
                u.vec = [comp[0, :u.cout_p], comp[1, :u.cout_p]] + u.vec[2:]
                nxt.fold_a = _FoldSource(self.pool[k], self.pool[k].shape[-1], u.vec[0], u.vec[1])
                dec.fold_a = _FoldSource(self.cat[k], self.cat[k].shape[-1], comp[0], comp[1])
            if p.head_fold:
                t = self.stages[-1]['tail']
                t.fold_b, u.apply_in_filters = u, True
                t.bias_fold = torch.zeros(t.cout_p, dtype=torch.float32, device=dev)
        for u in [c for c in convs if c.fold_a is not None]:
            u.cb = torch.zeros(9, u.cout_p, dtype=torch.float32, device=dev)
        nfw = max([lib.clamd_bn_fold_wgrad_workspace_bytes(B, u.cout_p) // 4 for u in convs if u.fold_a is not None] + [0])
        self.fold_ws = torch.empty(nfw, dtype=torch.float32, device=dev) if nfw else None
        self._tune_key = None
        self._plan_stat_rows()
        ws = 0
        for u in convs:
            ws = max(ws, lib.clamd_channel_sum_workspace_bytes(u.cout_p), u.g.wg_ws(lib, B, u.h, u.width, u.cout_p, u.cin_p, self.dcode),
                     ALGOS['igemm'].wg_ws(lib, B, u.h, u.width, u.cout_p, u.cin_p, self.dcode))
        for t in self.tails:
            mode = _lib.WGRAD_UP2 if t.kind == 'convT' else _lib.WGRAD_PW
            rp, cp_ = (t.cin_p, t.cout_p) if t.kind == 'convT' else (t.cout_p, t.cin_p)
            ws = max(ws, lib.clamd_wgrad_workspace_bytes(mode, B, H >> t.level, W >> t.level, rp, cp_, self.dcode))
        self.ws = torch.empty(ws // 4 + 16, dtype=torch.float32, device=dev)
        nvg = max([getattr(lib, u.d.x_elems)(B, u.h, u.width, u.cout_p) for u in convs if u.d is not None and u.d.pre] + [0])
        nyt = max([getattr(lib, u.g.wg_elems)(B, u.h, u.width, u.cout_p) for u in convs if u.g.pre] + [0])
        self.vg = torch.empty(nvg, dtype=torch.float32, device=dev) if nvg else None
        self.yt = torch.empty(nyt, dtype=torch.float32, device=dev) if nyt else None
        self.streams = _Streams(dev, bool(nyt or nfw))
        self.yt2 = torch.empty(nyt, dtype=torch.float32, device=dev) if (nyt and self.streams.x3 is not None) else None
        self.ws_bytes = ws
        self._build_pack_table()

    def _plan_stat_rows(self):
        key = tuple(self.tuning.as_dict().values())
        if key == self._tune_key:
            return
        self._tune_key = key
        B, dc, tn, lib = self.B, self.dcode, self.tuning, _lib.load()
        rows = _lib.stat_rows
        sizes, esz = [], []
        for u in self.convs:
            bb = u.f.border_bias
            u.fold_on = u.fold_a is not None and (bool(lib.clamd_conv3x3_border_bias_ok(B, u.h, u.width, u.cin_p, u.cout_p, dc, tune_ptr(tn)))
                                                  if bb is None else bb)
            if u.fold_a is not None:
                u.fold_a.apply_in_filters = u.fold_on
            u.gz_nrows = 0
            u.stat_rows = rows(u.f.stat_op, B, u.h, u.width, u.cin_p, u.cout_p, dc, tuning=tn)
            src = u.sum_src
            if src is None:
                u.sum_rows = rows(_lib.OP_BN_BWD_REDUCE, B, u.h, u.width, 1 if u.g_src[2] is not None else 0, u.cout_p, dc, tuning=tn)
            elif isinstance(src, _Unit):
                u.sum_rows = rows(src.d.stat_op, B, src.h, src.width, src.cout_p, src.cin_p, dc, fused_bn=True, tuning=tn)
                if lib.clamd_conv3x3_bn_sums(B, src.h, src.width, src.cout_p, src.cin_p, dc, tune_ptr(tn)) == 2:
                    u.gz_nrows = lib.clamd_bn_bwd_apply_sums_rows(B, u.h, u.width, u.cout_p)
            elif src.kind == 'head':
                u.sum_rows = rows(_lib.OP_CONV1X1, B, u.h, u.width, src.cout_p, src.cin_p, dc, fused_bn=True)
            else:
                u.sum_rows = rows(_lib.OP_CONVT2X2_DGRAD, B, u.h, u.width, src.cin_p, src.cout_p, dc, fused_bn=True)
            sizes.append((u.stat_rows * 2 + u.sum_rows * self.NS + u.gz_nrows) * u.cout_p)
            u.eval_nrows = 0 if u.fused_reduce else lib.clamd_bn_bwd_eval_rows(B, u.h, u.width, u.cout_p, 1 if u.g_src[2] is not None else 0)
            if u.eval_nrows < 0:
                _lib.check(u.eval_nrows, 'clamd_bn_bwd_eval_rows')
            esz.append(u.eval_nrows * 3 * u.cout_p)
        self.stat_arena = torch.empty(sum(sizes), dtype=torch.float32, device=self.dev)
        self.eval_arena = torch.empty(sum(esz), dtype=torch.float32, device=self.dev)
        off = eoff = 0
        for u, n, e in zip(self.convs, sizes, esz):
            k, k2 = u.stat_rows * 2 * u.cout_p, u.gz_nrows * u.cout_p
            u.stats = self.stat_arena[off:off + k]
            u.sums = self.stat_arena[off + k:off + n - k2]
            u.gz_rows = self.stat_arena[off + n - k2:off + n] if k2 else None
            u.eval_rows = self.eval_arena[eoff:eoff + e] if e else None
            off, eoff = off + n, eoff + e

    def _build_pack_table(self):
        tab = PackTable(self.dcode)
        late = PackTable(self.dcode)
        wtab = {(pl, late): WinoPackTable(pl) for pl in (16, 24, 36) for late in (False, True)}
        for i, u in enumerate(self.convs):
            u.pack_late = i >= 6
            if u.f.taps == 1:
                tab.head(u.w, u.wf, None, 9 * u.cin, u.cout)
            elif u.f.wino:
                if u.fold_a is None:
                    wtab[(u.f.taps, u.pack_late)].conv3x3(u.w, u.wf, None, u.cin_segs, u.cout)
                if u.wd is not None:
                    wtab[(u.d.taps, u.pack_late)].conv3x3(u.w, None, u.wd, u.cin_segs, u.cout)
            else:
                (late if u.pack_late else tab).conv3x3(u.w, None if u.fold_a is not None else u.wf, u.wd, u.cin_segs, u.cout)
            tab.vector(u.b, u.bias_p, u.cout)
            if u.fold_a is not None:
                u.fold_table, u.plain_table = [(WinoPackTable(u.f.taps) if u.f.wino else PackTable(self.dcode)) for _ in range(2)]
                u.fold_table.conv3x3(u.w, u.wf, None, u.cin_segs, u.cout, kscale=u.fold_a.vec[0])
                u.plain_table.conv3x3(u.w, u.wf, None, u.cin_segs, u.cout)
                u.fold_table.finalize(self.dev); u.plain_table.finalize(self.dev)
        for t in self.tails:
            if t.kind == 'convT':
                late.convT(t.w, t.wf, t.wd, t.cin, t.cout)
            elif t.fold_b is not None:
                late.head(t.w, None, t.wd, t.cin, t.cout)
                t.fold_table = PackTable(self.dcode)
                t.fold_table.head(t.w, t.wf, None, t.cin, t.cout, kscale=t.fold_b.vec[0])
                t.fold_table.finalize(self.dev)
            else:
                late.head(t.w, t.wf, t.wd, t.cin, t.cout)
            tab.vector(t.b, t.bias_p, t.cout)
        self.pack_table = tab.finalize(self.dev)
        self.pack_late = late.finalize(self.dev) if late.jobs else None
        self.wino_early = [t.finalize(self.dev) for (pl, late), t in wtab.items() if t.jobs and not late]
        self.wino_late = [t.finalize(self.dev) for (pl, late), t in wtab.items() if t.jobs and late]
        self._param_ptrs = [p.data_ptr() for p in self.model.parameters()]
# ... 163 lines not shown
        v = u.vec
        _hbm('bn_fwd', self.esize * self.B * u.h * u.width * u.cout * (9 if u.pooled is not None else 8) // 4,
             'clamd_bn_apply', ptr(u.y), u.cout_p, ptr(v[0]), ptr(v[1]), ptr(u.out), u.out_ldc,
             ptr(u.pooled), u.pooled.shape[-1] if u.pooled is not None else 0, self.B, u.h, u.width, u.cout_p, self.dcode, s)

    def backward(self, gout):
        m = self.model
        s = _lib.stream_ptr()
        B, H, W, dc = self.B, self.H, self.W, self.dcode
        if tuple(self.tuning.as_dict().values()) != self._tune_key:
            raise RuntimeError('model.tuning changed between forward and backward: change it between steps (before the forward)')
        if self.bn_group is not None and torch.cuda.is_current_stream_capturing():
            raise RuntimeError('UNet.backward: SyncBatchNorm layers in train mode all-reduce their sums, which a captured graph cannot do')
        p0 = next(iter(m.parameters()))
        if p0.grad is not None:
            lo = self.gflat.data_ptr()
            if lo <= p0.grad.data_ptr() < lo + 4 * self.gflat.numel():
                if m.grad_sync is not None:
                    raise RuntimeError('gradient accumulation (backward without zero_grad) is not supported together with '
                                       'ddp.GradSync: call optimizer.zero_grad() before every backward')
                self.gflat = torch.empty_like(self.gflat)
        base = self.gflat.data_ptr()
        g = {n: base + 4 * o for n, (o, _) in self.goffset.items()}
        sync, streams = m.grad_sync, self.streams
        streams.start_backward(sync is not None or self.bn_group is not None)
        if sync is not None:
            sync.begin()
        self._gp = g
        tp = tune_ptr(self.tuning)
        for st in reversed(self.stages):
            t = st.get('tail')
            if t is not None:
                h, w = H >> t.level, W >> t.level
                if t.kind == 'head':
                    src = self.dl_src
                    if not (src is not None and src[1:] == (gout.data_ptr(), gout._version, self.generation)):
                        call('clamd_nchw_to_nhwc', ptr(gout), ptr(self.dl), self.Kp, B, self.K, H, W, self.Kp, 1.0, dc, s)
                    self.dl_src = None
                    _hbm('head', self.esize * B * h * w * (self.Kp + t.cin),
                         'clamd_conv1x1', ptr(self.dl), self.Kp, ptr(t.wd), None, ptr(t.g_x), t.g_x.shape[-1], None,
                         *_sums_into(t.consumer), B, h, w, t.cout_p, t.cin_p, 0, dc, s)
                    sw = self.streams.param_grad_stream()
                    fb = t.fold_b
                    tx, tx_ldc = (fb.y, fb.cout_p) if fb is not None else (t.x, t.x.shape[-1])
                    _hbm('head', self.esize * B * h * w * (self.Kp + t.cin),
                         'clamd_wgrad', _lib.WGRAD_PW, ptr(self.dl), self.Kp, ptr(tx), tx_ldc, ptr(self.ws),
                         self.ws_bytes, g[t.keys[0]], B, h, w, t.cout_p, t.cin_p, t.cout, t.cin,
                         t.cout, t.cout_p, t.cin, t.cin_p, dc, tp, sw)
                    _hbm('head', 0,
                         'clamd_channel_sum', ptr(self.dl), self.Kp, g[t.keys[1]], B * h * w, self.Kp, t.cout, dc,
                         ptr(self.ws), self.ws_bytes, tp, sw)
                    if fb is not None:
                        call('clamd_bn_fold_wgrad_pointwise', g[t.keys[1]], ptr(fb.vec[0]), ptr(fb.vec[1]), g[t.keys[0]], t.cout, t.cin, sw)
                else:
                    ctb = self.esize * (B * h * w * (t.cin + 4 * t.cout) + 4 * t.cin * t.cout)
                    _hbm('convT', ctb,
                         'clamd_convT2x2_dgrad', ptr(t.gy_slice), t.y_ldc, ptr(t.wd), ptr(t.g_x), t.g_x.shape[-1],
                         *_sums_into(t.consumer), B, h, w, t.cin_p, t.cout_p, dc, s)
                    sw = self.streams.param_grad_stream()
                    _hbm('convT', ctb,
                         'clamd_wgrad', _lib.WGRAD_UP2, ptr(t.x), t.x.shape[-1], ptr(t.gy_slice), t.y_ldc, ptr(self.ws),
                         self.ws_bytes, g[t.keys[0]], B, h, w, t.cin_p, t.cout_p, t.cin, t.cout,
                         t.cin, t.cin_p, t.cout, t.cout_p, dc, tp, sw)
                    _hbm('convT', 0,
                         'clamd_channel_sum', ptr(t.gy_slice), t.y_ldc, g[t.keys[1]], B * 4 * h * w, t.cout_p,
                         t.cout, dc, ptr(self.ws), self.ws_bytes, tp, sw)
            for u in reversed(st['convs']):
                self._conv_bwd(u, s)
            if sync is not None:
                streams.join_stage()
                sync.stage_done(self, st)
        streams.join_backward()
        gf = self.gflat
        return [gf[o:o + k].view(self.gshape[n]) for n, (o, k) in ((n, self.goffset[n]) for n in self.param_names)]

    def _conv_bwd(self, u, s):
        B, dc, tp, streams = self.B, self.dcode, tune_ptr(self.tuning), self.streams
        v, g = u.vec, self._gp
        ga, ga_ldc, gp = u.g_src
        gp_ldc = gp.shape[-1] if gp is not None else 0
        count = float(B * u.h * u.width)
        dgamma, dbeta, dbias = g[u.keys[2]], g[u.keys[3]], g[u.keys[1]]
        two = u.fused_reduce and u.gz_nrows > 0
        if not u.bn_train and not u.fused_reduce:
            _hbm('bn_bwd', self.esize * B * u.h * u.width * u.cout * (13 if gp is not None else 12) // 4,
                 'clamd_bn_bwd_eval', ptr(ga), ga_ldc, ptr(gp), gp_ldc, ptr(u.y), u.y_ldc,
                 ptr(v[0]), ptr(v[1]), ptr(u.gz), u.cout_p, ptr(u.eval_rows), u.eval_nrows, B, u.h, u.width, u.cout_p, u.cout, dc, s)
            bnops.bwd_eval_finalize(u.eval_rows, u.eval_nrows, 3, v, False, dgamma, dbeta, dbias, u.cout_p, u.cout, streams.param_grad_stream())
        else:
            if not u.bn_train:
                bnops.bwd_eval_finalize(u.sums, u.sum_rows, self.NS, v, True, dgamma, dbeta, None if two else dbias, u.cout_p, u.cout, s)
            else:
                if not u.fused_reduce:
                    _hbm('bn_bwd', 0,
                         'clamd_bn_bwd_reduce', ptr(ga), ga_ldc, ptr(gp), gp_ldc, ptr(u.y), u.y_ldc,
                         ptr(v[0]), ptr(v[1]), ptr(u.sums), u.sum_rows, B, u.h, u.width, u.cout_p, dc, tp, s)
                bnops.bwd_finalize(u.sums, u.sum_rows, self.NS, u.gamma, v, dgamma, dbeta, None if two else dbias, u.cout_p, u.cout, count, s,
                                   (u.sync_tot, u.sync_red) if u.bn_sync else None, self.bn_group)
            if two:
                assert gp is None
                _hbm('bn_bwd', self.esize * B * u.h * u.width * u.cout * 3,
                     'clamd_bn_bwd_apply_sums', ptr(ga), ga_ldc, ptr(u.y), u.y_ldc, ptr(v[4]), ptr(u.gz), u.cout_p, ptr(u.gz_rows), u.gz_nrows,
                     B, u.h, u.width, u.cout_p, dc, s)
            else:
                _hbm('bn_bwd', self.esize * B * u.h * u.width * u.cout * (13 if gp is not None else 12) // 4,
                     'clamd_bn_bwd_apply', ptr(ga), ga_ldc, ptr(gp), gp_ldc, ptr(u.y), u.y_ldc,
                     ptr(v[0]), ptr(v[1]), ptr(v[4]), ptr(u.gz), u.cout_p, B, u.h, u.width, u.cout_p, dc, s)
        c_seg0, c_seg0p = u.cin_segs[0] if len(u.cin_segs) == 2 else (u.cin, u.cin_p)
        flops, nbytes = 2.0 * B * u.h * u.width * 9 * u.cin * u.cout, self._conv_bytes(u)
        gz_arg, yt = ptr(u.gz), self.yt
        if u.g.pre:
            sx, buf = streams.wgrad_transform_stream((self.yt, self.yt2))
            if sx is not None:
                call(u.g.wg_xform, gz_arg, u.cout_p, ptr(buf), B, u.h, u.width, u.cout_p, sx)
                streams.wgrad_transformed()
                gz_arg, yt = None, buf
        early = U.WGRAD_TAIL_EARLY and dc != _lib.BF16 and u.level == 0 and u.name.startswith('enc1')
        sw = streams.param_grad_stream() if early else None
        if u.d is not None:
            tag, gi = u.tag['dgrad'], u.g_in
            if u.d.pre:
                _timed('wino_transform', 0.0, u.d.x_bytes * B * u.h * u.width * u.cout_p, tag, u.d.xform, ptr(u.gz), u.cout_p, None, None, ptr(self.vg),
                       B, u.h, u.width, u.cout_p, s)
                _timed('igemm_conv3x3', flops, nbytes, tag, u.d.conv, ptr(self.vg), ptr(u.wd), None, ptr(gi), gi.shape[-1], None, 0,
                       B, u.h, u.width, u.cout_p, u.cin_p, 0, tp, s)
            elif u.d.wino:
                _timed('igemm_conv3x3', flops, nbytes, tag, u.d.conv, ptr(u.gz), u.cout_p, ptr(u.wd), None, ptr(gi), gi.shape[-1], None, 0,
                       B, u.h, u.width, u.cout_p, u.cin_p, 0, tp, s)
            else:
                _timed('igemm_conv3x3', flops, nbytes, tag, u.d.conv, ptr(u.gz), u.cout_p, ptr(u.wd), None, ptr(gi), gi.shape[-1], None,
                       *_sums_into(u.consumer), B, u.h, u.width, u.cout_p, u.cin_p, 0, 1 if 9 * u.cin_p > B * u.h * u.width else 0, dc, tp, s)
        if sw is None:
            sw = streams.param_grad_stream()
        if two:
            call('clamd_rows_sum', ptr(u.gz_rows), u.gz_nrows, dbias, u.cout_p, u.cout, sw)
        if u.g.taps == 1:
            _hbm('enc1.0', self.esize * B * u.h * u.width * (u.cout + u.cin_p),
                 u.g.wgrad, _lib.WGRAD_PW, ptr(u.gz), u.cout_p, ptr(u.xin), u.xin_ldc, ptr(self.ws), self.ws_bytes,
                 g[u.keys[0]], B, u.h, u.width, u.cout_p, u.cin_p, u.cout, 9 * u.cin, u.cout, u.cout_p, 9 * u.cin, u.cin_p, dc, tp, sw)
            return
        tag = u.tag['wgrad']
        xin, xin_ldc = (u.fold_a.y, u.fold_a.cout_p) if u.fold_on else (u.xin, u.xin_ldc)
        if u.g.pre:
            if gz_arg is None:
                streams.wgrad_after_transform()
            _timed('wgrad_conv3x3', flops, nbytes, tag, u.g.wgrad, gz_arg, u.cout_p, ptr(u.vx), ptr(yt), ptr(self.ws), self.ws_bytes,
                   g[u.keys[0]], B, u.h, u.width, u.cout_p, u.cin_p, u.cout, u.cin, u.cout, u.cout_p, c_seg0, c_seg0p, tp, sw)
            if gz_arg is None:
                streams.wgrad_operand_read()
        elif u.g.wino:
            _timed('wgrad_conv3x3', flops, nbytes, tag, u.g.wgrad, gz_arg, u.cout_p, ptr(xin), xin_ldc, ptr(self.ws), self.ws_bytes,
                   g[u.keys[0]], B, u.h, u.width, u.cout_p, u.cin_p, u.cout, u.cin, u.cout, u.cout_p, c_seg0, c_seg0p, tp, sw)
        else:
            _timed('wgrad_conv3x3', flops, nbytes, tag, u.g.wgrad, _lib.WGRAD_CONV3, gz_arg, u.cout_p, ptr(xin), xin_ldc, ptr(self.ws), self.ws_bytes,
                   g[u.keys[0]], B, u.h, u.width, u.cout_p, u.cin_p, u.cout, u.cin, u.cout, u.cout_p, c_seg0, c_seg0p, dc, tp, sw)
        if u.fold_on:
            a = u.fold_a
            call('clamd_bn_fold_wgrad', ptr(u.gz), u.cout_p, dbias, ptr(a.vec[0]), ptr(a.vec[1]), g[u.keys[0]], ptr(self.fold_ws),
                 4 * self.fold_ws.numel(), B, u.h, u.width, u.cout_p, u.cout, u.cin, dc, streams.fold_fixup_stream(sw))
```

### continual-learning_amd/plan.py

```python
from collections import namedtuple
from typing import NamedTuple, Optional

from . import _lib
from .ops import cpad


class Algo(NamedTuple):
    conv: str
    wgrad: str
    taps: int
    stat_op: int
    frac: float
    wg_ws: object
    border_bias: Optional[bool] = False
    bn_sums: bool = False
    xform: Optional[str] = None
    x_elems: Optional[str] = None
    x_bytes: int = 0
    wg_xform: Optional[str] = None
    wg_elems: Optional[str] = None

    wino = property(lambda a: a.taps > 9)
    pre = property(lambda a: a.xform is not None)


ALGOS = {
    'im2col': Algo('clamd_conv1x1', 'clamd_wgrad', 1, _lib.OP_CONV1X1, 1.0,
                   lambda lib, B, H, W, rp, cp, dc: lib.clamd_wgrad_workspace_bytes(_lib.WGRAD_PW, B, H, W, rp, cp, dc)),
    'igemm': Algo('clamd_conv3x3', 'clamd_wgrad', 9, _lib.OP_CONV3X3, 1.0,
                  lambda lib, B, H, W, rp, cp, dc: lib.clamd_wgrad_workspace_bytes(_lib.WGRAD_CONV3, B, H, W, rp, cp, dc), border_bias=None, bn_sums=True),
    'f22': Algo('clamd_conv3x3_winograd', 'clamd_wgrad_winograd', 16, _lib.OP_CONV3X3_WINOGRAD, 16 / 36,
                lambda lib, B, H, W, rp, cp, dc: lib.clamd_wgrad_winograd_workspace_bytes(rp, cp)),
    'f24': Algo('clamd_conv3x3_winograd24', 'clamd_wgrad_winograd24', 24, _lib.OP_CONV3X3_WINOGRAD24, 24 / 72,
                lambda lib, B, H, W, rp, cp, dc: lib.clamd_wgrad_winograd24_workspace_bytes(rp, cp), border_bias=True),
    'f24_direct': Algo('clamd_conv3x3_winograd24_direct_filters', None, 24, _lib.OP_CONV3X3_WINOGRAD24, 24 / 72, None, border_bias=True),
    'f24_pre': Algo('clamd_conv3x3_winograd24_pre', 'clamd_wgrad_winograd24_pre', 24, _lib.OP_CONV3X3_WINOGRAD24, 24 / 72,
                    lambda lib, B, H, W, rp, cp, dc: lib.clamd_wgrad_winograd24_pre_workspace_bytes(B, H, W, rp, cp),
                    xform='clamd_winograd24_transform_input', x_elems='clamd_winograd24_input_elems', x_bytes=16,
                    wg_xform='clamd_wgrad_winograd24_pre_transform', wg_elems='clamd_wgrad_winograd24_pre_operand_elems'),
    'f44_pre': Algo('clamd_conv3x3_winograd44_pre', 'clamd_wgrad_winograd44_pre', 36, _lib.OP_CONV3X3_WINOGRAD44, 36 / 144,
                    lambda lib, B, H, W, rp, cp, dc: lib.clamd_wgrad_winograd44_pre_workspace_bytes(B, H, W, rp, cp),
                    xform='clamd_winograd44_transform_input', x_elems='clamd_winograd44_input_elems', x_bytes=13,
                    wg_xform='clamd_wgrad_winograd44_pre_transform', wg_elems='clamd_wgrad_winograd44_pre_operand_elems'),
}
F24 = ('f24', 'f24_direct')

Switches = namedtuple('Switches', 'WINOGRAD WINOGRAD24 WINOGRAD24_WGRAD PRETRANSFORM WINOGRAD44 NARROW_DIRECT NARROW_PRE_WGRAD '
                                 'FOLD_BN_INTO_TRANSFORM FOLD_BN_INTO_FILTERS FOLD_FILTERS_MAX_CHANNELS FOLD_POOLED FUSE_BN_SUMS')


Unit = namedtuple('Unit', 'name level h w cin_segs cin_p cout cout_p fwd dgrad wgrad sums_by fold_src fold_a pool_fold head_fold',
                  defaults=(None, None, None, None, False))


def _choose(lib, sw, B, h, w, cin_segs, cout_p, first, dcode, ncu):
    cin, cin_p = sum(s[0] for s in cin_segs), sum(s[1] for s in cin_segs)
    if first and 9 * cin <= cpad(9 * cin) == cin_p:
        return 'im2col', None, 'im2col'
    if not (sw.WINOGRAD and dcode == _lib.F32 and (h | w) % 2 == 0 and min(h, w) >= 8):
        return 'igemm', None if first else 'igemm', 'igemm'
    if not (sw.WINOGRAD24 and w % 4 == 0):
        return 'f22', None if first else 'f22', 'f22'
    wg24 = min(h, w) >= 64 if sw.WINOGRAD24_WGRAD == 'auto' else bool(sw.WINOGRAD24_WGRAD)
    items24 = B * ((h + 7) // 8 * ((w + 31) // 32) if w >= 32 else (h + 15) // 16 * ((w + 15) // 16)) * ((cin_p + 63) // 64)
    dg24 = not (2 * items24 <= ncu)
    pt = sw.PRETRANSFORM
    blocks44 = B * h * w // 512
    ok44 = lambda slab_ch, in_ch: (bool(sw.WINOGRAD44) and h % 4 == 0 and w % 4 == 0 and slab_ch % 64 == 0
                                   and (sw.WINOGRAD44 is True or blocks44 * (slab_ch // 64) >= ncu)
                                   and lib.clamd_winograd44_input_elems(B, h, w, in_ch) * 4 < (1 << 32))
    wg_pre = bool(pt) and cin_p % 256 == 0 and cout_p % 256 == 0
    fwd_pre = bool(pt) and cin_p >= 64 and cout_p % 64 == 0 and (
        pt is True or (cin_p >= 256 and (wg_pre or 2 * cout_p > cin_p)) or (cin_p >= 128 and cout_p >= 2 * cin_p))
    fits = lambda c: lib.clamd_winograd24_input_elems(B, h, w, c) * 4 < (1 << 32)
    fwd_pre = fwd_pre and fits(cin_p)
    wg_pre = wg_pre and fwd_pre and lib.clamd_wgrad_winograd24_pre_operand_elems(B, h, w, cout_p) * 4 // 24 < (1 << 32)
    dg_pre = bool(pt) and dg24 and not first and cout_p >= 64 and cin_p % 64 == 0 and fits(cout_p) and (
        pt is True or (cout_p >= 256 and (2 * cin_p > cout_p or (2 * cin_p == cout_p and cin_p >= 256))))
    if (pt == 'auto' and sw.WINOGRAD44 and not (fwd_pre and wg_pre) and min(cin_p, cout_p) >= 128
            and cin_p % 128 == 0 and cout_p % 128 == 0 and ok44(cout_p, cin_p) and sw.NARROW_PRE_WGRAD):
        fwd_pre = wg_pre = True
    fwd44 = fwd_pre and ok44(cout_p, cin_p)
    if (pt == 'auto' and not dg_pre and dg24 and not first and cin_p >= 128 and cout_p >= 64 and cin_p % 64 == 0
            and sw.WINOGRAD44 and ok44(cin_p, cout_p)):
        dg_pre = True
    dg44 = dg_pre and ok44(cin_p, cout_p)
    if fwd44 and wg_pre:
        wg_pre = lib.clamd_wgrad_winograd44_pre_operand_elems(B, h, w, cout_p) * 4 // 36 < (1 << 32)
    fwd_narrow = sw.NARROW_DIRECT and not fwd_pre and cin_p == 64 and cout_p % 64 == 0
    dg_narrow = sw.NARROW_DIRECT and dg24 and not dg_pre and cout_p == 64 and cin_p % 64 == 0
    fpre = 'f44_pre' if fwd44 else 'f24_pre'
    fwd = fpre if fwd_pre else ('f24_direct' if fwd_narrow else 'f24')
    dgrad = None if first else (('f44_pre' if dg44 else 'f24_pre') if dg_pre else ('f24_direct' if dg_narrow else ('f24' if dg24 else 'f22')))
    return fwd, dgrad, (fpre if wg_pre else ('f24' if wg24 else 'f22'))


def plan_net(table, B, H, W, dcode, sw, ncu=256):
    lib = _lib.load()
    units = []
    for i, st in enumerate(table):
        level, pre = (i if i < 4 else 8 - i), st['name'] + ('.block' if st['wrapped'] else '')
        (c0, _, cin, mid), (c1, _, _, _) = st['convs']
        segs = ((cin // 2, cpad(cin // 2)),) * 2 if i > 4 else ((cin, cpad(cin)),)
        for ci, segs in ((c0, segs), (c1, ((mid, cpad(mid)),))):
            h, w, first = H >> level, W >> level, i == 0 and ci == c0
            fwd, dgrad, wgrad = _choose(lib, sw, B, h, w, segs, cpad(mid), first, dcode, ncu)
            units.append(dict(name=f'{pre}.{ci}', level=level, h=h, w=w, cin_segs=segs, cin_p=sum(s[1] for s in segs), cout=mid,
                              cout_p=cpad(mid), fwd=fwd, dgrad=dgrad, wgrad=wgrad))
        a, b = units[-2:]
        auto = dcode == _lib.BF16 and b['cout_p'] <= 256 and b['cout_p'] % 64 == 0
        if ALGOS[b['dgrad']].bn_sums and (auto if sw.FUSE_BN_SUMS == 'auto' else sw.FUSE_BN_SUMS):
            a['sums_by'] = b['name']
        if st['tail'] is not None and sw.FUSE_BN_SUMS is True:
            b['sums_by'] = f"{pre}.{st['tail'][1]}"
        if sw.FOLD_BN_INTO_TRANSFORM and ALGOS[b['fwd']].pre and ALGOS[b['wgrad']].pre:
            b['fold_src'] = a['name']
        elif sw.FOLD_BN_INTO_FILTERS and not ALGOS[b['fwd']].pre and min(b['h'], b['w']) >= 2 and b['cin_p'] <= sw.FOLD_FILTERS_MAX_CHANNELS:
            b['fold_a'] = a['name']
        if st['tail'] is not None and st['tail'][0] == 'head' and sw.FOLD_BN_INTO_FILTERS and b['cout_p'] <= sw.FOLD_FILTERS_MAX_CHANNELS:
            b['head_fold'] = True
    for k in range(3):
        b, nxt, dec = units[2 * k + 1], units[2 * k + 2], units[2 * (8 - k)]
        if (sw.FOLD_POOLED and sw.FOLD_BN_INTO_FILTERS and dcode == _lib.F32 and b['fwd'] in F24 and b['cout'] == b['cout_p']
                and all(c['fwd'] in F24 and c['cin_p'] <= sw.FOLD_FILTERS_MAX_CHANNELS and all(lg == ph for lg, ph in c['cin_segs'])
                        for c in (nxt, dec))):
            b['pool_fold'] = (nxt['name'], dec['name'])
    return tuple(Unit(**u) for u in units)
```

### continual-learning_amd/unet.py

```python
import math
import os
import weakref

import torch
import torch.nn as nn

from . import _lib
from .ops import cpad
from .plan import Switches


def _env_tri(name):
    return {'0': False, 'false': False, '1': True, 'true': True}.get(os.environ.get(name, 'auto').lower(), 'auto')


def _env_flag(name, default=True):
    v = _env_tri(name)
    return default if v == 'auto' else v


FUSE_BN_SUMS = _env_tri('CLAMD_FUSE_BN_SUMS')

WINOGRAD = True
WINOGRAD24 = True
WINOGRAD24_WGRAD = 'auto'
PRETRANSFORM = _env_tri('CLAMD_PRETRANSFORM')
WINOGRAD44 = _env_tri('CLAMD_WINOGRAD44')
FOLD_BN_INTO_TRANSFORM = _env_flag('CLAMD_FOLD_BN')
NARROW_DIRECT = _env_flag('CLAMD_NARROW_DIRECT')
WGRAD_TAIL_EARLY = _env_flag('CLAMD_WGRAD_TAIL_EARLY')
NARROW_PRE_WGRAD = _env_flag('CLAMD_NARROW_PRE_WGRAD')
FOLD_BN_INTO_FILTERS = _env_flag('CLAMD_FOLD_FILTERS')
FOLD_FILTERS_MAX_CHANNELS = int(os.environ.get('CLAMD_FOLD_FILTERS_MAX_CHANNELS', '128'))
FOLD_POOLED = _env_flag('CLAMD_FOLD_POOLED')
WGRAD_XFORM_STREAM = _env_flag('CLAMD_WGRAD_XFORM_STREAM')
WGRAD_STREAM = _env_flag('CLAMD_WGRAD_STREAM')
PACK_LATE_STREAM = _env_flag('CLAMD_PACK_LATE_STREAM')
PACK_LATE_AT = int(os.environ.get('CLAMD_PACK_LATE_AT', '2'))

KERNEL_TIMING = None


def switches():
    return Switches(*(globals()[k] for k in Switches._fields))


def stage_table(num_classes, in_dim=3, conv_dim=64):
    d = conv_dim
    t = [dict(name='enc1', wrapped=False, pool=False, convs=[(0, 2, in_dim, d), (3, 5, d, d)], tail=None)]
    c = d
    for i in (2, 3, 4):
        t.append(dict(name=f'enc{i}', wrapped=True, pool=True, convs=[(1, 3, c, 2 * c), (4, 6, 2 * c, 2 * c)], tail=None))
        c *= 2
    for i, (cin, mid, cout) in enumerate([(8 * d, 16 * d, 8 * d), (16 * d, 8 * d, 4 * d), (8 * d, 4 * d, 2 * d),
                                          (4 * d, 2 * d, d)], 1):
        t.append(dict(name=f'dec{i}', wrapped=True, pool=False, convs=[(0, 2, cin, mid), (3, 5, mid, mid)],
                      tail=('convT', 6, mid, cout)))
    t.append(dict(name='last', wrapped=False, pool=False, convs=[(0, 2, 2 * d, d), (3, 5, d, d)],
                  tail=('head', 6, d, num_classes)))
    return t


class _NoForward:

    def forward(self, *args, **kwargs):
        raise RuntimeError(f'{type(self).__name__}.forward: the layers of continual-learning_amd.UNet only hold parameters; '
                           'run UNet.forward / UNet.predict, or a whole block (model.enc2(x), model.dec1(x): blocks.py) -- there is no '
                           'stock-torch path for a single layer')


class _Seq(_NoForward, nn.Sequential):
    def forward(self, x):
        spec = getattr(self, '_block_spec', None)
        if spec is None:
            return _NoForward.forward(self, x)
        from . import blocks
        return blocks.run_block(self, spec[0], spec[1], x)


class _Conv2d(_NoForward, nn.Conv2d):
    pass


class _ConvTranspose2d(_NoForward, nn.ConvTranspose2d):
    pass


class _BatchNorm2d(_NoForward, nn.BatchNorm2d):
    pass


class _ReLU(_NoForward, nn.ReLU):
    pass


class _MaxPool2d(_NoForward, nn.MaxPool2d):
    pass


class _Stage(_NoForward, nn.Module):

    def __init__(self, layers):
        super().__init__()
        self.block = _Seq(*layers)

    def forward(self, x):
        return self.block(x)


def _stage_modules(st):
    layers = [_MaxPool2d(2, 2)] if st['pool'] else []
    for _, _, cin, cout in st['convs']:
        layers += [_Conv2d(cin, cout, 3, 1, 1), _ReLU(), _BatchNorm2d(cout)]
    if st['tail'] is not None:
        kind, _, cin, cout = st['tail']
        layers.append(_ConvTranspose2d(cin, cout, 2, 2) if kind == 'convT' else _Conv2d(cin, cout, 1, 1))
    return layers

# ... 124 lines not shown
```

### include/clamd.h

```cpp
#ifndef CLAMD_H
#define CLAMD_H
#include <stddef.h>

#ifdef __cplusplus
extern "C" {
#endif

enum { CLAMD_F32 = 0, CLAMD_BF16 = 1, CLAMD_SPLIT = 2 };
enum { CLAMD_WGRAD_CONV3 = 0, CLAMD_WGRAD_PW = 1, CLAMD_WGRAD_UP2 = 2 };

const char* clamd_last_error(void);
int clamd_version(void);
int clamd_sizeof_pack_job(void);
int clamd_sizeof_adam_tensor(void);
int clamd_adam_chunk_elems(void);
int clamd_sizeof_importance_tensor(void);
int clamd_pack_tile(void);
int clamd_bn_bwd_nsums(void);

typedef struct clamd_tuning {
    int igemm_pws, igemm_ws, igemm_variant, pws_wres;
    int wgrad_ws, wgrad_dma, wgrad_xcd, wgrad_blocks, wgrad_tw16;
    int wino_band, wino_persist, wino_mt;
    int bn_reduce_blocks, chsum_blocks;
// ... 18 lines not shown
int clamd_bn_fold_bias(const float* w, const float* shift, const float* bias, float* table, int Cout, int Cin, int Cout_p, void* stream);
int clamd_bn_fold_pack(int form, const void* jobs_dev, int njobs, int total_blocks, int dtype, const float* w, int taps, const float* shift,
                       const float* bias, float* table, int Cout, int Cin, int Cout_p, void* stream);
int clamd_bn_fold_wgrad_pointwise(const float* sum_g, const float* scale, const float* shift, float* dw, int Cout, int Cin, void* stream);
size_t clamd_bn_fold_wgrad_workspace_bytes(int B, int Cout_p);
int clamd_bn_fold_wgrad(const void* gz, int gz_ldc, const float* sum_gz, const float* scale, const float* shift, float* dw,
                        void* workspace, size_t ws_bytes, int B, int H, int W, int Cout_p, int Cout, int Cin, int dtype, void* stream);
int clamd_sizeof_wino_pack_job(void);
int clamd_wino_pack(const void* jobs_dev, int njobs, int total_blocks, void* stream);
int clamd_conv3x3_winograd(const float* x, int x_ldc, const float* w_wino, const float* bias, float* y, int y_ldc,
                           float* stats, int stat_rows, int B, int H, int W, int Cin_p, int Cout_p, int relu,
                           const clamd_tuning* tune, void* stream);
int clamd_wino24_pack(const void* jobs_dev, int njobs, int total_blocks, void* stream);
int clamd_conv3x3_winograd24(const float* x, int x_ldc, const float* w_wino, const float* bias, float* y, int y_ldc,
                             float* stats, int stat_rows, int B, int H, int W, int Cin_p, int Cout_p, int relu,
                             const clamd_tuning* tune, void* stream);
size_t clamd_wgrad_winograd24_workspace_bytes(int Rp, int Cp);
int clamd_wgrad_winograd24(const float* gz, int gz_ldc, const float* x, int x_ldc, float* workspace, size_t ws_bytes, float* out,
                           int B, int H, int W, int Rp, int Cp, int R, int C, int r_seg0, int r_seg0p, int c_seg0, int c_seg0p,
                           const clamd_tuning* tune, void* stream);
size_t clamd_winograd24_input_elems(int B, int H, int W, int Cp);
int clamd_winograd24_transform_input(const float* x, int x_ldc, const float* scale, const float* shift, float* v, int B, int H, int W,
                                     int Cp, void* stream);
int clamd_conv3x3_winograd24_pre(const float* v, const float* w_wino, const float* bias, float* y, int y_ldc,
                                 float* stats, int stat_rows, int B, int H, int W, int Cin_p,
                                 int Cout_p, int relu, const clamd_tuning* tune, void* stream);
int clamd_conv3x3_winograd24_direct_filters(const float* x, int x_ldc, const float* w_wino, const float* bias, float* y, int y_ldc,
                                            float* stats, int stat_rows, int B, int H, int W,
                                            int Cin_p, int Cout_p, int relu, const clamd_tuning* tune, void* stream);
size_t clamd_wgrad_winograd24_pre_operand_elems(int B, int H, int W, int Rp);
int clamd_wgrad_winograd24_pre_transform(const float* gz, int gz_ldc, float* yt, int B, int H, int W, int Rp, void* stream);
size_t clamd_wgrad_winograd24_pre_workspace_bytes(int B, int H, int W, int Rp, int Cp);
int clamd_wgrad_winograd24_pre(const float* gz, int gz_ldc, const float* v, float* yt, float* workspace, size_t ws_bytes, float* out,
                               int B, int H, int W, int Rp, int Cp, int R, int C, int r_seg0, int r_seg0p, int c_seg0, int c_seg0p,
                               const clamd_tuning* tune, void* stream);
int clamd_wino44_pack(const void* jobs_dev, int njobs, int total_blocks, void* stream);
size_t clamd_winograd44_input_elems(int B, int H, int W, int Cp);
int clamd_winograd44_transform_input(const float* x, int x_ldc, const float* scale, const float* shift, float* v, int B, int H, int W,
                                     int Cp, void* stream);
int clamd_conv3x3_winograd44_pre(const float* v, const float* w_wino, const float* bias, float* y, int y_ldc,
                                 float* stats, int stat_rows, int B, int H, int W, int Cin_p,
                                 int Cout_p, int relu, const clamd_tuning* tune, void* stream);
size_t clamd_wgrad_winograd44_pre_operand_elems(int B, int H, int W, int Rp);
int clamd_wgrad_winograd44_pre_transform(const float* gz, int gz_ldc, float* yt, int B, int H, int W, int Rp, void* stream);
size_t clamd_wgrad_winograd44_pre_workspace_bytes(int B, int H, int W, int Rp, int Cp);
int clamd_wgrad_winograd44_pre(const float* gz, int gz_ldc, const float* v, float* yt, float* workspace, size_t ws_bytes, float* out,
                               int B, int H, int W, int Rp, int Cp, int R, int C, int r_seg0, int r_seg0p, int c_seg0, int c_seg0p,
                               const clamd_tuning* tune, void* stream);
size_t clamd_wgrad_winograd_workspace_bytes(int Rp, int Cp);
int clamd_wgrad_winograd(const float* gz, int gz_ldc, const float* x, int x_ldc, float* workspace, size_t ws_bytes, float* out,
                         int B, int H, int W, int Rp, int Cp, int R, int C, int r_seg0, int r_seg0p, int c_seg0, int c_seg0p,
                         const clamd_tuning* tune, void* stream);
int clamd_conv1x1(const void* x, int x_ldc, const void* w_packed, const float* bias, void* y, int y_ldc,
                  float* stats, const void* bn_y, float* bn_sums, int stat_rows, int B, int H, int W, int Cin_p, int Cout_p,
                  int relu, int dtype, void* stream);
int clamd_conv1x1_logits(const void* x, int x_ldc, const void* w_packed, const float* bias, float* logits_nchw,
                         int B, int H, int W, int Cin_p, int Cout_p, int num_classes, int dtype, void* stream);
int clamd_conv1x1_argmax(const void* x, int x_ldc, const void* w_packed, const float* bias, long long* pred, float* logits_nchw,
                         int B, int H, int W, int Cin_p, int Cout_p, int num_classes, int dtype, void* stream);
int clamd_convT2x2_fwd(const void* x, int x_ldc, const void* w_packed, const float* bias, void* y, int y_ldc, int B,
                       int h, int w, int Cin_p, int Cout_p, int dtype, void* stream);
int clamd_convT2x2_dgrad(const void* gy, int gy_ldc, const void* w_packed, void* gx, int gx_ldc, const void* bn_y,
                         float* bn_sums, int stat_rows, int B, int h, int w, int Cin_p, int Cout_p, int dtype, void* stream);

size_t clamd_wgrad_workspace_bytes(int mode, int B, int H, int W, int Rp, int Cp, int dtype);
int clamd_wgrad(int mode, const void* a, int a_ldc, const void* b, int b_ldc, float* workspace, size_t ws_bytes,
                float* out, int B, int H, int W, int Rp, int Cp, int R, int C, int r_seg0, int r_seg0p, int c_seg0,
                int c_seg0p, int dtype, const clamd_tuning* tune, void* stream);

int clamd_bn_finalize(const float* stats, int stat_rows, const float* gamma, const float* beta, float* running_mean,
                      float* running_var, float* scale, float* shift, float* save_mean, float* save_istd,
                      int Cp, int C, double count, double momentum, double eps, long long* num_batches_tracked, void* stream);
int clamd_bn_apply(const void* y, int y_ldc, const float* scale, const float* shift, void* out, int out_ldc,
                   void* pooled, int p_ldc, int B, int H, int W, int Cp, int dtype, void* stream);
int clamd_bn_bwd_reduce(const void* ga, int ga_ldc, const void* gp, int gp_ldc, const void* y, int y_ldc,
                        const float* scale, const float* shift, float* sums, int sum_rows, int B, int H, int W, int Cp,
                        int dtype, const clamd_tuning* tune, void* stream);
int clamd_bn_bwd_finalize(const float* sums, int sum_rows, const float* gamma, const float* save_mean, const float* save_istd,
                          float* k012, float* dgamma, float* dbeta, float* dbias, int Cp, int C, double count,
                          void* stream);
int clamd_bn_bwd_apply(const void* ga, int ga_ldc, const void* gp, int gp_ldc, const void* y, int y_ldc,
                       const float* scale, const float* shift, const float* k012, void* gz, int gz_ldc, int B,
                       int H, int W, int Cp, int dtype, void* stream);
int clamd_bn_bwd_apply_sums_rows(int B, int H, int W, int Cp);
int clamd_bn_bwd_apply_sums(const void* ga, int ga_ldc, const void* y, int y_ldc, const float* k012, void* gz, int gz_ldc,
                            float* gz_rows, int nrows, int B, int H, int W, int Cp, int dtype, void* stream);
int clamd_rows_sum(const float* rows, int nrows, float* out, int Cp, int C, void* stream);
int clamd_bn_bwd_eval_rows(int B, int H, int W, int Cp, int pooled);
int clamd_bn_bwd_eval(const void* ga, int ga_ldc, const void* gp, int gp_ldc, const void* y, int y_ldc, const float* scale, const float* shift,
                      void* gz, int gz_ldc, float* rows, int nrows, int B, int H, int W, int Cp, int C, int dtype, void* stream);
int clamd_bn_bwd_eval_finalize(const float* rows, int nrows, int nsums, const float* scale, const float* save_mean, const float* save_istd,
                               float* k012, float* dgamma, float* dbeta, float* dbias, int Cp, int C, void* stream);
int clamd_bn_rows_total(const float* rows, int nrows, int nk, int Cp, double count, double* totals, double* reduce, void* stream);
int clamd_bn_finalize_total(const double* reduce, const float* gamma, const float* beta, float* running_mean, float* running_var,
                            float* scale, float* shift, float* save_mean, float* save_istd, int Cp, int C, double momentum, double eps,
                            long long* num_batches_tracked, void* stream);
int clamd_bn_bwd_finalize_total(const double* totals, const double* reduce, const float* gamma, const float* save_mean,
                                const float* save_istd, float* k012, float* dgamma, float* dbeta, float* dbias, int Cp, int C, void* stream);
int clamd_maxpool2x2(const void* x, int x_ldc, const float* sign, void* pooled, int p_ldc, int B, int H, int W, int Cp, int dtype, void* stream);
int clamd_maxpool2x2_bwd(const void* x, int x_ldc, const float* sign, const void* gp, int gp_ldc, void* gx, int gx_ldc, int B, int H, int W, int Cp,
                         int dtype, void* stream);
size_t clamd_channel_sum_workspace_bytes(int Cp);
int clamd_channel_sum(const void* g, int ldc, float* out, long long npix, int Cp, int C, int dtype, float* workspace,
                      size_t ws_bytes, const clamd_tuning* tune, void* stream);
int clamd_nchw_to_nhwc(const float* src, void* dst, int ldc, int B, int C, int H, int W, int Cp, double mul,
                       int dtype, void* stream);
int clamd_nhwc_to_nchw(const void* src, int ldc, float* dst, int B, int C, int H, int W, int dtype, void* stream);
int clamd_nchw_im2col3(const float* src, void* dst, int ldc, int B, int C, int H, int W, int Cp, int dtype, void* stream);

int clamd_pack(const void* jobs_dev, int njobs, int total_blocks, int dtype, void* stream);
size_t clamd_ce_workspace_bytes(void);
size_t clamd_ce_bad_label_count_offset(void);
int clamd_ce_fwd_bwd(const float* logits, const long long* labels, const float* old_logits, int K_old_total, int c_old,
                     double temperature, double lam, float* dlogits, float* loss3, void* workspace, size_t ws_bytes,
                     int B, int K, int H, int W, long long ignore_index, double grad_scale, void* stream);
int clamd_ce_count(const long long* labels, int B, int K, int H, int W, long long ignore_index, void* workspace, size_t ws_bytes, void* stream);
int clamd_ce_fwd_bwd_counted(const float* logits, const long long* labels, float* dlogits, void* dl_nhwc, int dl_ldc, int dl_dtype,
                             float* loss3, void* workspace, size_t ws_bytes, int B, int K, int H, int W, long long ignore_index,
                             double grad_scale, void* stream);
int clamd_ce_unbiased_fwd_bwd(const float* logits, const long long* labels, const float* old_logits, int K_old_total, int c_old, double lam,
                              float* dlogits, void* dl_nhwc, int dl_ldc, int dl_dtype, float* loss3, void* workspace, size_t ws_bytes,
                              int B, int K, int H, int W, long long ignore_index, double grad_scale, void* stream);
size_t clamd_ce_dice_workspace_bytes(int B, int K, int H, int W, int per_image);
int clamd_ce_dice_fwd_bwd(const float* logits, const long long* labels, float* dlogits, void* dl_nhwc, int dl_ldc, int dl_dtype,
                          float* loss3, void* workspace, size_t ws_bytes, int B, int K, int H, int W, long long ignore_index,
                          double w_ce, double w_dice, double smooth, int first_class, int present_only, int per_image,
                          double grad_scale, void* stream);
int clamd_pseudo_entropy_hist(const float* old_logits, int K_old_total, int c_old, const long long* labels, long long* hist, int nbins,
                              int B, int H, int W, void* stream);
int clamd_pseudo_label(const float* old_logits, int K_old_total, int c_old, const long long* labels_in, const float* thresholds,
                       long long* labels_out, unsigned int* counts, float* image_weight, double min_factor, int B, int H, int W,
                       long long ignore_index, void* stream);
int clamd_ce_fwd_bwd_weighted(const float* logits, const long long* labels, const float* image_weight, float* dlogits, void* dl_nhwc,
                              int dl_ldc, int dl_dtype, float* loss3, void* workspace, size_t ws_bytes, int B, int K, int H, int W,
                              long long ignore_index, double grad_scale, void* stream);
size_t clamd_pod_workspace_bytes(int B, int C, int H, int W, int levels);
int clamd_local_pod_fwd_bwd(const float* a, int Ca, const float* b, int Cb, int C, int merge_extra, int square, int normalize,
                            int levels, double lam, float* da, float* loss1, void* workspace, size_t ws_bytes,
                            int B, int H, int W, double grad_scale, void* stream);
int clamd_class_pixel_counts(const long long* labels, int* counts, unsigned int* bad, int B, int K, int H, int W, long long ignore_index,
                             void* stream);
int clamd_replay_store(const float* images, const long long* labels, const int* src, const int* slot, int n, void* store_images,
                       unsigned char* store_labels, int store_fp32, int cap, unsigned int* bad, int B, int C, int H, int W, int K,
                       long long ignore_index, void* stream);
int clamd_replay_mix(const float* cur_images, const long long* cur_labels, int B, const void* store_images, const unsigned char* store_labels,
                     int store_fp32, int cap, const long long* slots, const int* flips, int R, float* out_images, long long* out_labels,
                     unsigned int* bad, int C, int H, int W, long long ignore_index, void* stream);
int clamd_augment_batch(const float* images, const long long* labels, const long long* params, int B, int C, int H, int W,
                        float* out_images, long long* out_labels, double fill, long long ignore_index, unsigned int* bad, void* stream);
int clamd_adam_step(const void* tensors_dev, const void* chunks_dev, int nchunks, const float* hyper_dev, int* step_dev,
                    float* derived_dev, float* l2_accum_dev, void* stream);
int clamd_adam_step_consolidated(const void* tensors_dev, const void* importance_dev, const void* chunks_dev, int nchunks,
                                 const float* hyper_dev, int* step_dev, float* derived_dev, float* ewc_accum_dev, float* l2_accum_dev,
                                 void* stream);
int clamd_importance_accum(const void* tensors_dev, const void* chunks_dev, int nchunks, double decay, double scale, int power, void* stream);
int clamd_sizeof_sgd_tensor(void);
int clamd_sgd_step(const void* tensors_dev, const void* importance_dev, const void* chunks_dev, int nchunks, const float* hyper_dev,
                   float* ewc_accum_dev, float* l2_accum_dev, void* stream);
int clamd_adam_step_tracked(const void* tensors_dev, const void* importance_dev, const void* path_dev, const void* chunks_dev, int nchunks,
                            const float* hyper_dev, int* step_dev, float* derived_dev, float* ewc_accum_dev, float* l2_accum_dev,
                            void* stream);
int clamd_sgd_step_tracked(const void* tensors_dev, const void* importance_dev, const void* path_dev, const void* chunks_dev, int nchunks,
                           const float* hyper_dev, float* ewc_accum_dev, float* l2_accum_dev, void* stream);
int clamd_sizeof_path_tensor(void);
int clamd_path_importance(const void* tensors_dev, const void* chunks_dev, int nchunks, double decay, double xi, void* stream);
int clamd_argmax_confusion(const float* logits, const long long* labels, long long* pred, unsigned long long* conf,
// ... 16 lines not shown
```

Before: 848.4 images/sec.

## Fuse BN backward apply with Winograd wgrad operand transform

```diff
diff --git a/continual-learning_amd/_lib.py b/continual-learning_amd/_lib.py
--- a/continual-learning_amd/_lib.py
+++ b/continual-learning_amd/_lib.py
@@ -70,6 +70,8 @@
     'clamd_bn_bwd_reduce': (_I, [_P, _I, _P, _I, _P, _I, _P, _P, _P, _I, _I, _I, _I, _I, _I, _P, _P]),
     'clamd_bn_bwd_finalize': (_I, [_P, _I, _P, _P, _P, _P, _P, _P, _P, _I, _I, _D, _P]),
     'clamd_bn_bwd_apply': (_I, [_P, _I, _P, _I, _P, _I, _P, _P, _P, _P, _I, _I, _I, _I, _I, _I, _P]),
+    'clamd_bn_bwd_apply_wgxform44': (_I, [_P, _I, _P, _I, _P, _I, _P, _P, _P, _P, _I, _P, _I, _I, _I, _I, _I, _I, _I, _P]),
+    'clamd_bn_bwd_apply_wgxform24': (_I, [_P, _I, _P, _I, _P, _I, _P, _P, _P, _P, _I, _P, _I, _I, _I, _I, _I, _I, _I, _P]),
     'clamd_bn_bwd_apply_sums_rows': (_I, [_I, _I, _I, _I]),
     'clamd_bn_bwd_apply_sums': (_I, [_P, _I, _P, _I, _P, _P, _I, _P, _I, _I, _I, _I, _I, _I, _P]),
     'clamd_rows_sum': (_I, [_P, _I, _P, _I, _I, _P]),
diff --git a/continual-learning_amd/csrc/elementwise.hip b/continual-learning_amd/csrc/elementwise.hip
--- a/continual-learning_amd/csrc/elementwise.hip
+++ b/continual-learning_amd/csrc/elementwise.hip
@@ -2,6 +2,7 @@
 #include <type_traits>
 #include "common.hip.h"
 #include "clamd_internal.h"
+#include "wino_common.hip.h"
 
 namespace clamd {
 
@@ -218,6 +219,22 @@
     }
 }
 
+template <int N>
+__device__ inline void pool_arg_step(int q, const float (&yq)[N], const float (&sc)[N], const float (&sh)[N], float (&best)[N], int (&arg)[N]) {
+#pragma unroll
+    for (int j = 0; j < N; ++j) {
+        float u = __fmaf_rn(yq[j], sc[j], sh[j]);
+        if (q == 0 || u > best[j]) { best[j] = u; arg[j] = q; }
+    }
+}
+template <int N>
+__device__ inline void pool_route(const int (&arg)[N], const float (&gpv)[N], float (&g)[4][N]) {
+#pragma unroll
+    for (int q = 0; q < 4; ++q)
+#pragma unroll
+        for (int j = 0; j < N; ++j) g[q][j] += (arg[j] == q) ? gpv[j] : 0.f;
+}
+
 template <typename T>
 __device__ inline void load_gu(const T* ga, int ga_ldc, const T* gp, int gp_ldc, const T* y, int y_ldc,
                                const float (&sc)[8], const float (&sh)[8], const PoolWindow& win,
@@ -233,18 +250,11 @@
 #pragma unroll
             for (int j = 0; j < 8; ++j) g[q][j] = 0.f;
         }
-#pragma unroll
-        for (int j = 0; j < 8; ++j) {
-            float u = __fmaf_rn(yy[q][j], sc[j], sh[j]);
-            if (q == 0 || u > best[j]) { best[j] = u; arg[j] = q; }
-        }
+        pool_arg_step<8>(q, yy[q], sc, sh, best, arg);
     }
     float gpv[8];
     Vec8<T>::load(gp + win.cell() * gp_ldc + cg * 8, gpv);
-#pragma unroll
-    for (int q = 0; q < 4; ++q)
-#pragma unroll
-        for (int j = 0; j < 8; ++j) g[q][j] += (arg[j] == q) ? gpv[j] : 0.f;
+    pool_route<8>(arg, gpv, g);
 }
 
 constexpr int NSUM = 5;
@@ -430,6 +440,130 @@
     }
 }
 
+struct ApplyWgxParams {
+    const float* ga; int ga_ldc;
+    const float* gp; int gp_ldc;
+    const float* y; int y_ldc;
+    const float* scale; const float* shift; const float* k012;
+    float* gz; int gz_ldc;
+    float* yt;
+    int B, H, W, Cp, Tp;
+};
+
+__device__ inline void ld4(__amdgpu_buffer_rsrc_t rs, unsigned off, float (&v)[4]) {
+    const uint4 u = buf_ld16(rs, off, 0u);
+    v[0] = __uint_as_float(u.x); v[1] = __uint_as_float(u.y); v[2] = __uint_as_float(u.z); v[3] = __uint_as_float(u.w);
+}
+
+template <int TH, int TXN, bool POOL>
+__global__ void __launch_bounds__(256) bn_bwd_apply_wgxform_kernel(const ApplyWgxParams p) {
+    PASS_PRIO();
+    constexpr int TYN = 32 / TXN, PW = 4 * TXN, PH = TH * TYN, NI = TH == 4 ? 6 : 4;
+    const int ng = p.Cp >> 2;
+    const long long total = (long long)p.Tp * ng;
+    const int tiles_x = (p.W + PW - 1) / PW, tiles_y = (p.H + PH - 1) / PH;
+    const unsigned hw = (unsigned)p.H * (unsigned)p.W;
+    const unsigned ga_img = p.ga ? hw * (unsigned)p.ga_ldc * 4u : 0u, y_img = hw * (unsigned)p.y_ldc * 4u, gz_img = hw * (unsigned)p.gz_ldc * 4u;
+    const unsigned gp_img = POOL ? (hw >> 2) * (unsigned)p.gp_ldc * 4u : 0u;
+    const size_t ps = (size_t)p.Tp * p.Cp;
+    for (long long idx = (long long)blockIdx.x * 256 + threadIdx.x; idx < total; idx += (long long)gridDim.x * 256) {
+        const int g = (int)(idx % ng);
+        const int t = (int)(idx / ng);
+        const int tm = t >> 5, r = t & 31;
+        const int x0 = (tm % tiles_x) * PW + 4 * (r % TXN), y0 = ((tm / tiles_x) % tiles_y) * PH + TH * (r / TXN), b = tm / (tiles_x * tiles_y);
+        const bool inside = b < p.B && y0 < p.H && x0 < p.W;
+        const int bi = inside ? b : 0;
+        float* const dst = p.yt + (size_t)t * p.Cp + 4 * g;
+        const __amdgpu_buffer_rsrc_t ars = make_rsrc((const char*)p.ga + (size_t)bi * ga_img, ga_img);
+        const __amdgpu_buffer_rsrc_t yrs = make_rsrc((const char*)p.y + (size_t)bi * y_img, y_img);
+        const __amdgpu_buffer_rsrc_t zrs = make_rsrc((char*)p.gz + (size_t)bi * gz_img, gz_img);
+        const float4 k0 = *reinterpret_cast<const float4*>(p.k012 + 4 * g), k1 = *reinterpret_cast<const float4*>(p.k012 + p.Cp + 4 * g),
+                     k2 = *reinterpret_cast<const float4*>(p.k012 + 2 * p.Cp + 4 * g);
+        const float kk0[4] = {k0.x, k0.y, k0.z, k0.w}, kk1[4] = {k1.x, k1.y, k1.z, k1.w}, kk2[4] = {k2.x, k2.y, k2.z, k2.w};
+        float z[NI][4][4];
+#pragma unroll
+        for (int qp = 0; qp < 2; ++qp) {
+            float gq[TH][2][4];
+            if constexpr (POOL) {
+                const float4 s4 = *reinterpret_cast<const float4*>(p.scale + 4 * g), h4 = *reinterpret_cast<const float4*>(p.shift + 4 * g);
+                const float sc[4] = {s4.x, s4.y, s4.z, s4.w}, sh[4] = {h4.x, h4.y, h4.z, h4.w};
+                const __amdgpu_buffer_rsrc_t prs = make_rsrc((const char*)p.gp + (size_t)bi * gp_img, gp_img);
+#pragma unroll
+                for (int wy = 0; wy < TH / 2; ++wy) {
+                    float gu[4][4], yy[4][4], best[4], gpv[4];
+                    int arg[4];
+#pragma unroll
+                    for (int m = 0; m < 4; ++m) {
+                        const int py = y0 + 2 * wy + (m >> 1), px = x0 + 2 * qp + (m & 1);
+                        const unsigned pix = (unsigned)(py * p.W + px);
+                        ld4(yrs, inside ? (pix * (unsigned)p.y_ldc + 4u * g) * 4u : BUF_OOB, yy[m]);
+                        ld4(ars, inside ? (pix * (unsigned)p.ga_ldc + 4u * g) * 4u : BUF_OOB, gu[m]);
+                        pool_arg_step<4>(m, yy[m], sc, sh, best, arg);
+                    }
+                    const unsigned cell = (unsigned)(((y0 >> 1) + wy) * (p.W >> 1) + (x0 >> 1) + qp);
+                    ld4(prs, inside ? (cell * (unsigned)p.gp_ldc + 4u * g) * 4u : BUF_OOB, gpv);
+                    pool_route<4>(arg, gpv, gu);
+#pragma unroll
+                    for (int m = 0; m < 4; ++m) {
+                        float (&o)[4] = gq[2 * wy + (m >> 1)][m & 1];
+#pragma unroll
+                        for (int e = 0; e < 4; ++e) o[e] = yy[m][e] > 0.f ? bn_bwd_gz(kk0[e], kk1[e], kk2[e], gu[m][e], yy[m][e]) : 0.f;
+                    }
+                }
+            } else {
+#pragma unroll
+                for (int c = 0; c < 2; ++c)
+#pragma unroll
+                    for (int a = 0; a < TH; ++a) {
+                        const unsigned pix = (unsigned)((y0 + a) * p.W + x0 + 2 * qp + c);
+                        float gu[4], yy[4];
+                        ld4(ars, inside ? (pix * (unsigned)p.ga_ldc + 4u * g) * 4u : BUF_OOB, gu);
+                        ld4(yrs, inside ? (pix * (unsigned)p.y_ldc + 4u * g) * 4u : BUF_OOB, yy);
+#pragma unroll
+                        for (int e = 0; e < 4; ++e) gq[a][c][e] = yy[e] > 0.f ? bn_bwd_gz(kk0[e], kk1[e], kk2[e], gu[e], yy[e]) : 0.f;
+                    }
+            }
+#pragma unroll
+            for (int a = 0; a < TH; ++a)
+#pragma unroll
+                for (int c = 0; c < 2; ++c) {
+                    const unsigned pix = (unsigned)((y0 + a) * p.W + x0 + 2 * qp + c);
+                    buf_st16(zrs, inside ? (pix * (unsigned)p.gz_ldc + 4u * g) * 4u : BUF_OOB, 0u,
+                             make_uint4(__float_as_uint(gq[a][c][0]), __float_as_uint(gq[a][c][1]), __float_as_uint(gq[a][c][2]), __float_as_uint(gq[a][c][3])));
+                }
+#pragma unroll
+            for (int c = 0; c < 2; ++c)
+#pragma unroll
+                for (int e = 0; e < 4; ++e) {
+                    if constexpr (TH == 4) {
+                        const float col[4] = {gq[0][c][e], gq[1][c][e], gq[2][c][e], gq[3][c][e]};
+                        float o[6];
+                        w44_a6(col, o);
+#pragma unroll
+                        for (int i = 0; i < 6; ++i) z[i][2 * qp + c][e] = o[i];
+                    } else {
+#pragma unroll
+                        for (int i = 0; i < 4; ++i) z[i][2 * qp + c][e] = w24_a4(i, gq[0][c][e], gq[1][c][e]);
+                    }
+                }
+        }
+#pragma unroll
+        for (int i = 0; i < NI; ++i) {
+            float o[6][4];
+#pragma unroll
+            for (int e = 0; e < 4; ++e) {
+                const float row[4] = {z[i][0][e], z[i][1][e], z[i][2][e], z[i][3][e]};
+                float oo[6];
+                w44_a6(row, oo);
+#pragma unroll
+                for (int j = 0; j < 6; ++j) o[j][e] = oo[j];
+            }
+#pragma unroll
+            for (int j = 0; j < 6; ++j) *reinterpret_cast<float4*>(dst + (6 * i + j) * ps) = make_float4(o[j][0], o[j][1], o[j][2], o[j][3]);
+        }
+    }
+}
+
 template <typename T>
 __global__ void __launch_bounds__(256) bn_bwd_apply_sums_kernel(const T* __restrict__ ga, int ga_ldc, const T* __restrict__ y, int y_ldc,
                                                                 const float* __restrict__ k012, T* gz, int gz_ldc, float* rows,
@@ -802,6 +936,38 @@
     return 0;
 }
 
+template <int TH>
+static int launch_apply_wgxform(const char* name, const void* ga, int ga_ldc, const void* gp, int gp_ldc, const void* y, int y_ldc, const float* scale,
+                                const float* shift, const float* k012, void* gz, int gz_ldc, float* yt, int B, int H, int W, int Cp, int Rp,
+                                int Tp, int dtype, void* stream) {
+    const Need pool_only = gp ? REQUIRED : OPTIONAL;
+    if (int e = check_streaming(name, pow2_channels(Cp), POW2_RULE, Cp, B, H, W, gp != nullptr, dtype,
+                                {{ga, ga_ldc, SOURCE}, {gp, gp_ldc, SOURCE}, {y, y_ldc, REQUIRED}, {k012, NO_PITCH, REQUIRED},
+                                 {gz, gz_ldc, REQUIRED}, {yt, NO_PITCH, REQUIRED}, {scale, NO_PITCH, pool_only}, {shift, NO_PITCH, pool_only}}))
+        return e;
+    if (dtype != CLAMD_F32) return fail(name, "fp32 only (the pre-transformed weight gradients are fp32 kernels)");
+    if ((H % TH) || (W & 3)) return fail(name, TH == 4 ? "H and W must be multiples of 4" : "H must be even and W a multiple of 4");
+    const WinoTile tile = TH == 4 ? w44_block(W) : w24_tile(W);
+    const long long tiles = wino_tiles(tile, B, H, W) * 32;
+    if (Rp != Cp || Tp != tiles) return fail(name, "Rp must be Cp and Tp the tile count of the operand (32 per tile block)");
+    if ((ga && ga_ldc % 4) || (gp && gp_ldc % 4) || y_ldc % 4 || gz_ldc % 4) return fail(name, "pitches must be multiples of 4");
+    const long long hw = (long long)H * W, top = std::max({ga ? ga_ldc : 0, y_ldc, gz_ldc, gp ? (gp_ldc + 3) / 4 : 0});
+    if (hw * top * 4 >= (1ll << 31)) return fail(name, "one image exceeds 2^31 bytes");
+    if (tiles * Rp * 4 >= (1ll << 32)) return fail(name, "one plane of the operand exceeds 2^32 bytes");
+    const long long na = (tiles * (Cp / 4) + 255) / 256;
+    const dim3 grid((unsigned)std::min<long long>(na, 1 << 20)), block(256);
+    const ApplyWgxParams p{(const float*)ga, ga_ldc, (const float*)gp, gp_ldc, (const float*)y, y_ldc, scale, shift, k012, (float*)gz, gz_ldc, yt,
+                           B, H, W, Cp, Tp};
+    auto pick = [](bool b, auto&& f) { if (b) f(std::true_type{}); else f(std::false_type{}); };
+    pick(W >= 32, [&](auto wide) {
+        pick(gp != nullptr, [&](auto pool) {
+            hipLaunchKernelGGL((bn_bwd_apply_wgxform_kernel<TH, decltype(wide)::value ? 8 : 4, decltype(pool)::value>), grid, block, 0,
+                               (hipStream_t)stream, p);
+        });
+    });
+    return clamd_check_launch(name);
+}
+
 extern "C" {
 
 int clamd_bn_finalize(const float* stats, int stat_rows, const float* gamma, const float* beta, float* running_mean,
@@ -937,6 +1103,20 @@
     return ok ? clamd_check_launch("bn_bwd_apply") : fail("bn_bwd_apply", "bad dtype");
 }
 
+int clamd_bn_bwd_apply_wgxform44(const void* ga, int ga_ldc, const void* gp, int gp_ldc, const void* y, int y_ldc, const float* scale,
+                                 const float* shift, const float* k012, void* gz, int gz_ldc, float* yt, int B, int H, int W, int Cp, int Rp,
+                                 int Tp, int dtype, void* stream) {
+    return launch_apply_wgxform<4>("bn_bwd_apply_wgxform44", ga, ga_ldc, gp, gp_ldc, y, y_ldc, scale, shift, k012, gz, gz_ldc, yt, B, H, W, Cp, Rp,
+                                   Tp, dtype, stream);
+}
+
+int clamd_bn_bwd_apply_wgxform24(const void* ga, int ga_ldc, const void* gp, int gp_ldc, const void* y, int y_ldc, const float* scale,
+                                 const float* shift, const float* k012, void* gz, int gz_ldc, float* yt, int B, int H, int W, int Cp, int Rp,
+                                 int Tp, int dtype, void* stream) {
+    return launch_apply_wgxform<2>("bn_bwd_apply_wgxform24", ga, ga_ldc, gp, gp_ldc, y, y_ldc, scale, shift, k012, gz, gz_ldc, yt, B, H, W, Cp, Rp,
+                                   Tp, dtype, stream);
+}
+
 static long long apply_sums_rows(long long npix, int Cp) { return grid_rows(npix * (Cp / 8), 256, 2048); }
 
 int clamd_bn_bwd_apply_sums_rows(int B, int H, int W, int Cp) {
diff --git a/continual-learning_amd/csrc/wino24g.hip b/continual-learning_amd/csrc/wino24g.hip
--- a/continual-learning_amd/csrc/wino24g.hip
+++ b/continual-learning_amd/csrc/wino24g.hip
@@ -637,17 +637,15 @@
             }
 #pragma unroll
         for (int i = 0; i < 4; ++i) {
-            float z[4][4], o[6][4];
-#pragma unroll
-            for (int q = 0; q < 4; ++q)
-#pragma unroll
-                for (int e = 0; e < 4; ++e)
-                    z[q][e] = i == 0 ? gq[0][q][e] : (i == 1 ? gq[0][q][e] + gq[1][q][e] : (i == 2 ? gq[0][q][e] - gq[1][q][e] : -gq[1][q][e]));
+            float o[6][4];
 #pragma unroll
             for (int e = 0; e < 4; ++e) {
-                const float sa = z[0][e] + z[2][e], sb = z[1][e] + z[3][e], sc = fmaf(4.f, z[2][e], z[0][e]), sd = fmaf(4.f, z[3][e], z[1][e]);
-                o[0][e] = z[0][e]; o[1][e] = sa + sb; o[2][e] = sa - sb;
-                o[3][e] = fmaf(2.f, sd, sc); o[4][e] = fmaf(-2.f, sd, sc); o[5][e] = z[3][e];
+                const float z[4] = {w24_a4(i, gq[0][0][e], gq[1][0][e]), w24_a4(i, gq[0][1][e], gq[1][1][e]),
+                                    w24_a4(i, gq[0][2][e], gq[1][2][e]), w24_a4(i, gq[0][3][e], gq[1][3][e])};
+                float oo[6];
+                w44_a6(z, oo);
+#pragma unroll
+                for (int j = 0; j < 6; ++j) o[j][e] = oo[j];
             }
 #pragma unroll
             for (int j = 0; j < 6; ++j) *reinterpret_cast<float4*>(dst + (6 * i + j) * ps) = make_float4(o[j][0], o[j][1], o[j][2], o[j][3]);
diff --git a/continual-learning_amd/csrc/wino44g.hip b/continual-learning_amd/csrc/wino44g.hip
--- a/continual-learning_amd/csrc/wino44g.hip
+++ b/continual-learning_amd/csrc/wino44g.hip
@@ -22,11 +22,6 @@
     o[1] = pq + qq; o[2] = pq - qq;
     o[3] = fmaf(2.f, ss, rr); o[4] = fmaf(-2.f, ss, rr);
     o[5] = fmaf(4.f, t[1], fmaf(-5.f, t[3], t[5]));
-}
-__device__ inline void w44_a6(const float (&z)[4], float (&o)[6]) {
-    const float sa = z[0] + z[2], sb = z[1] + z[3], sc = fmaf(4.f, z[2], z[0]), sd = fmaf(4.f, z[3], z[1]);
-    o[0] = z[0]; o[1] = sa + sb; o[2] = sa - sb;
-    o[3] = fmaf(2.f, sd, sc); o[4] = fmaf(-2.f, sd, sc); o[5] = z[3];
 }
 __device__ inline void w44_gt6(const float (&t)[6], float (&o)[3]) {
     const float s12 = t[1] + t[2], d12 = t[2] - t[1], s34 = t[3] + t[4], d34 = t[3] - t[4];
diff --git a/continual-learning_amd/csrc/wino_common.hip.h b/continual-learning_amd/csrc/wino_common.hip.h
--- a/continual-learning_amd/csrc/wino_common.hip.h
+++ b/continual-learning_amd/csrc/wino_common.hip.h
@@ -33,6 +33,13 @@
     const int l = seg0 + (p - seg0p);
     return l < L ? l : -1;
 }
+
+__device__ inline void w44_a6(const float (&z)[4], float (&o)[6]) {
+    const float sa = z[0] + z[2], sb = z[1] + z[3], sc = fmaf(4.f, z[2], z[0]), sd = fmaf(4.f, z[3], z[1]);
+    o[0] = z[0]; o[1] = sa + sb; o[2] = sa - sb;
+    o[3] = fmaf(2.f, sd, sc); o[4] = fmaf(-2.f, sd, sc); o[5] = z[3];
+}
+__device__ inline float w24_a4(int i, float g0, float g1) { return i == 0 ? g0 : (i == 1 ? g0 + g1 : (i == 2 ? g0 - g1 : -g1)); }
 
 struct WinoReduceParams {
     const float* partial; float* out;
diff --git a/continual-learning_amd/engine.py b/continual-learning_amd/engine.py
--- a/continual-learning_amd/engine.py
+++ b/continual-learning_amd/engine.py
@@ -204,7 +204,17 @@
     def wgrad_after_transform(self):
         self.wg.wait_event(self._x3_ev)
 
+    def wgrad_operand_buffer(self, bufs):
+        if self._single():
+            return bufs[0]
+        self._yt_flip ^= 1
+        if self._yt_ev[self._yt_flip] is not None:
+            torch.cuda.current_stream().wait_event(self._yt_ev[self._yt_flip])
+        return bufs[self._yt_flip]
+
     def wgrad_operand_read(self):
+        if self._single():
+            return
         self._yt_ev[self._yt_flip], self._x3_ev = torch.cuda.Event(), None
         self._yt_ev[self._yt_flip].record(self.wg)
 
@@ -393,7 +403,8 @@
         self.vg = torch.empty(nvg, dtype=torch.float32, device=dev) if nvg else None
         self.yt = torch.empty(nyt, dtype=torch.float32, device=dev) if nyt else None
         self.streams = _Streams(dev, bool(nyt or nfw))
-        self.yt2 = torch.empty(nyt, dtype=torch.float32, device=dev) if (nyt and self.streams.x3 is not None) else None
+        two_bufs = self.streams.x3 is not None or (self.streams.wg is not None and any(u.plan.wg_by_apply for u in convs))
+        self.yt2 = torch.empty(nyt, dtype=torch.float32, device=dev) if (nyt and two_bufs) else None
         self.ws_bytes = ws
         self._build_pack_table()
 
@@ -723,6 +734,7 @@
         count = float(B * u.h * u.width)
         dgamma, dbeta, dbias = g[u.keys[2]], g[u.keys[3]], g[u.keys[1]]
         two = u.fused_reduce and u.gz_nrows > 0
+        yt_by_apply = None
         if not u.bn_train and not u.fused_reduce:
             _hbm('bn_bwd', self.esize * B * u.h * u.width * u.cout * (13 if gp is not None else 12) // 4,
                  'clamd_bn_bwd_eval', ptr(ga), ga_ldc, ptr(gp), gp_ldc, ptr(u.y), u.y_ldc,
@@ -743,6 +755,12 @@
                 _hbm('bn_bwd', self.esize * B * u.h * u.width * u.cout * 3,
                      'clamd_bn_bwd_apply_sums', ptr(ga), ga_ldc, ptr(u.y), u.y_ldc, ptr(v[4]), ptr(u.gz), u.cout_p, ptr(u.gz_rows), u.gz_nrows,
                      B, u.h, u.width, u.cout_p, dc, s)
+            elif u.plan.wg_by_apply and u.bn_train and not u.bn_sync:
+                yt_by_apply = streams.wgrad_operand_buffer((self.yt, self.yt2))
+                tp_ = getattr(_lib.load(), u.g.wg_elems)(B, u.h, u.width, u.cout_p) // (u.g.taps * u.cout_p)
+                _hbm('bn_bwd', self.esize * B * u.h * u.width * u.cout * (13 if gp is not None else 12) // 4,
+                     u.g.wg_apply, ptr(ga), ga_ldc, ptr(gp), gp_ldc, ptr(u.y), u.y_ldc, ptr(v[0]), ptr(v[1]), ptr(v[4]), ptr(u.gz), u.cout_p,
+                     ptr(yt_by_apply), B, u.h, u.width, u.cout_p, u.cout_p, tp_, dc, s)
             else:
                 _hbm('bn_bwd', self.esize * B * u.h * u.width * u.cout * (13 if gp is not None else 12) // 4,
                      'clamd_bn_bwd_apply', ptr(ga), ga_ldc, ptr(gp), gp_ldc, ptr(u.y), u.y_ldc,
@@ -750,7 +768,9 @@
         c_seg0, c_seg0p = u.cin_segs[0] if len(u.cin_segs) == 2 else (u.cin, u.cin_p)
         flops, nbytes = 2.0 * B * u.h * u.width * 9 * u.cin * u.cout, self._conv_bytes(u)
         gz_arg, yt = ptr(u.gz), self.yt
-        if u.g.pre:
+        if yt_by_apply is not None:
+            gz_arg, yt = None, yt_by_apply
+        elif u.g.pre:
             sx, buf = streams.wgrad_transform_stream((self.yt, self.yt2))
             if sx is not None:
                 call(u.g.wg_xform, gz_arg, u.cout_p, ptr(buf), B, u.h, u.width, u.cout_p, sx)
@@ -783,7 +803,7 @@
         tag = u.tag['wgrad']
         xin, xin_ldc = (u.fold_a.y, u.fold_a.cout_p) if u.fold_on else (u.xin, u.xin_ldc)
         if u.g.pre:
-            if gz_arg is None:
+            if gz_arg is None and yt_by_apply is None:
                 streams.wgrad_after_transform()
             _timed('wgrad_conv3x3', flops, nbytes, tag, u.g.wgrad, gz_arg, u.cout_p, ptr(u.vx), ptr(yt), ptr(self.ws), self.ws_bytes,
                    g[u.keys[0]], B, u.h, u.width, u.cout_p, u.cin_p, u.cout, u.cin, u.cout, u.cout_p, c_seg0, c_seg0p, tp, sw)
diff --git a/continual-learning_amd/plan.py b/continual-learning_amd/plan.py
--- a/continual-learning_amd/plan.py
+++ b/continual-learning_amd/plan.py
@@ -19,6 +19,7 @@
     x_bytes: int = 0
     wg_xform: Optional[str] = None
     wg_elems: Optional[str] = None
+    wg_apply: Optional[str] = None
 
     wino = property(lambda a: a.taps > 9)
     pre = property(lambda a: a.xform is not None)
@@ -37,20 +38,22 @@
     'f24_pre': Algo('clamd_conv3x3_winograd24_pre', 'clamd_wgrad_winograd24_pre', 24, _lib.OP_CONV3X3_WINOGRAD24, 24 / 72,
                     lambda lib, B, H, W, rp, cp, dc: lib.clamd_wgrad_winograd24_pre_workspace_bytes(B, H, W, rp, cp),
                     xform='clamd_winograd24_transform_input', x_elems='clamd_winograd24_input_elems', x_bytes=16,
-                    wg_xform='clamd_wgrad_winograd24_pre_transform', wg_elems='clamd_wgrad_winograd24_pre_operand_elems'),
+                    wg_xform='clamd_wgrad_winograd24_pre_transform', wg_elems='clamd_wgrad_winograd24_pre_operand_elems',
+                    wg_apply='clamd_bn_bwd_apply_wgxform24'),
     'f44_pre': Algo('clamd_conv3x3_winograd44_pre', 'clamd_wgrad_winograd44_pre', 36, _lib.OP_CONV3X3_WINOGRAD44, 36 / 144,
                     lambda lib, B, H, W, rp, cp, dc: lib.clamd_wgrad_winograd44_pre_workspace_bytes(B, H, W, rp, cp),
                     xform='clamd_winograd44_transform_input', x_elems='clamd_winograd44_input_elems', x_bytes=13,
-                    wg_xform='clamd_wgrad_winograd44_pre_transform', wg_elems='clamd_wgrad_winograd44_pre_operand_elems'),
+                    wg_xform='clamd_wgrad_winograd44_pre_transform', wg_elems='clamd_wgrad_winograd44_pre_operand_elems',
+                    wg_apply='clamd_bn_bwd_apply_wgxform44'),
 }
 F24 = ('f24', 'f24_direct')
 
 Switches = namedtuple('Switches', 'WINOGRAD WINOGRAD24 WINOGRAD24_WGRAD PRETRANSFORM WINOGRAD44 NARROW_DIRECT NARROW_PRE_WGRAD '
-                                 'FOLD_BN_INTO_TRANSFORM FOLD_BN_INTO_FILTERS FOLD_FILTERS_MAX_CHANNELS FOLD_POOLED FUSE_BN_SUMS')
+                                 'FOLD_BN_INTO_TRANSFORM FOLD_BN_INTO_FILTERS FOLD_FILTERS_MAX_CHANNELS FOLD_POOLED FUSE_BN_SUMS APPLY_WGXFORM')
 
 
-Unit = namedtuple('Unit', 'name level h w cin_segs cin_p cout cout_p fwd dgrad wgrad sums_by fold_src fold_a pool_fold head_fold',
-                  defaults=(None, None, None, None, False))
+Unit = namedtuple('Unit', 'name level h w cin_segs cin_p cout cout_p fwd dgrad wgrad sums_by fold_src fold_a pool_fold head_fold wg_by_apply',
+                  defaults=(None, None, None, None, False, False))
 
 
 def _choose(lib, sw, B, h, w, cin_segs, cout_p, first, dcode, ncu):
@@ -125,4 +128,7 @@
                 and all(c['fwd'] in F24 and c['cin_p'] <= sw.FOLD_FILTERS_MAX_CHANNELS and all(lg == ph for lg, ph in c['cin_segs'])
                         for c in (nxt, dec))):
             b['pool_fold'] = (nxt['name'], dec['name'])
+    on = dcode == _lib.F32 if sw.APPLY_WGXFORM == 'auto' else (bool(sw.APPLY_WGXFORM) and dcode == _lib.F32)
+    for u in units:
+        u['wg_by_apply'] = bool(on and ALGOS[u['wgrad']].pre and u.get('sums_by') is None)
     return tuple(Unit(**u) for u in units)
diff --git a/continual-learning_amd/unet.py b/continual-learning_amd/unet.py
--- a/continual-learning_amd/unet.py
+++ b/continual-learning_amd/unet.py
@@ -34,6 +34,7 @@
 FOLD_FILTERS_MAX_CHANNELS = int(os.environ.get('CLAMD_FOLD_FILTERS_MAX_CHANNELS', '128'))
 FOLD_POOLED = _env_flag('CLAMD_FOLD_POOLED')
 WGRAD_XFORM_STREAM = _env_flag('CLAMD_WGRAD_XFORM_STREAM')
+APPLY_WGXFORM = _env_tri('CLAMD_APPLY_WGXFORM')
 WGRAD_STREAM = _env_flag('CLAMD_WGRAD_STREAM')
 PACK_LATE_STREAM = _env_flag('CLAMD_PACK_LATE_STREAM')
 PACK_LATE_AT = int(os.environ.get('CLAMD_PACK_LATE_AT', '2'))
diff --git a/include/clamd.h b/include/clamd.h
--- a/include/clamd.h
+++ b/include/clamd.h
@@ -124,6 +124,12 @@
 int clamd_bn_bwd_apply(const void* ga, int ga_ldc, const void* gp, int gp_ldc, const void* y, int y_ldc,
                        const float* scale, const float* shift, const float* k012, void* gz, int gz_ldc, int B,
                        int H, int W, int Cp, int dtype, void* stream);
+int clamd_bn_bwd_apply_wgxform44(const void* ga, int ga_ldc, const void* gp, int gp_ldc, const void* y, int y_ldc, const float* scale,
+                                 const float* shift, const float* k012, void* gz, int gz_ldc, float* yt, int B, int H, int W, int Cp, int Rp,
+                                 int Tp, int dtype, void* stream);
+int clamd_bn_bwd_apply_wgxform24(const void* ga, int ga_ldc, const void* gp, int gp_ldc, const void* y, int y_ldc, const float* scale,
+                                 const float* shift, const float* k012, void* gz, int gz_ldc, float* yt, int B, int H, int W, int Cp, int Rp,
+                                 int Tp, int dtype, void* stream);
 int clamd_bn_bwd_apply_sums_rows(int B, int H, int W, int Cp);
 int clamd_bn_bwd_apply_sums(const void* ga, int ga_ldc, const void* y, int y_ldc, const float* k012, void* gz, int gz_ldc,
                             float* gz_rows, int nrows, int B, int H, int W, int Cp, int dtype, void* stream);
```

Measured after the change: 852.1 images/sec (median of 6 runs). About the same (+0.4%).
